# youngers2006/Dreamer

Hardware: AMD Instinct MI355X
Metric: imagined latent-steps/sec (B×H) at 64×64 CarRacing, 1/2/4/8 MI355X (higher is better)
Workload: dtype f32; 1 GPU; Dreamer.train_Agent() with AC_epochs=1 (replay sample + warm start S/2 + H-step imagination + actor-critic update), B=256/GPU S=64 H=15 64x64x3, precision=fp32 (north-star batch per GPU); global_batch=256, seq_len=64, horizon=15, parallelism=dp1, precision=fp32

## Files before the change

dreamer_amd/csrc/engine.hip:

```cpp
#include "engine_util.h"
#include "scan.h"
#include "dream.h"
#include "bptt.h"


static bool s3_first_layer(const dr_dims* d, int M, int N, const float* h, long long ldh, const float* z,
                           long long ldz) {
  return d->precision != DR_PREC_BF16 && M >= 1024 && ldh < INT_MAX && ldz < INT_MAX &&
         op_gemm_nt_split3_supported(M, N, d->hidden + latent(d), h, (int)ldh, z, (int)ldz, d->hidden, N);
}

struct EncWs {
  float *x0, *a[DR_MAX_DEPTH], *wr[DR_MAX_DEPTH], *sk;
  long long sk_n;
  void* wproj;
  void* s3proj;
  float* s3part;
  size_t s3part_n;
};

static void enc_carve(Carve& c, const dr_dims* d, int n, EncWs& w) {
  memset(&w, 0, sizeof(w));
  if (d->obs_dim > 0) {
    const int F = enc_feat_dim(d);
// ... 230 lines not shown
  WS_CHECK(c, ws_bytes);
  const int L = latent(d), Hd = d->hidden, eh = d->enc_hidden;
  const int F = enc_feat_dim(d);
  const bool any_gru = (z_init != nullptr) || T > 1;
  if (any_gru) {
    DR_REQUIRE(wm->w_ih && wm->w_hh && wm->b_ih && wm->b_hh, "GRU weights required");
    DR_TRY(op_transpose(3 * Hd, L + d->action, wm->w_ih, w.wt, s));
  }
  if (z_init == nullptr && h_init == nullptr && op_pscan_supported(d, B, T, d->action)) {
    const int rc = op_pscan(d, wm, B, T, d->action, feat, actions, act_sb, act_st, w.wt, wm->map0.w + F, F + Hd,
                            noise, 0, z_out, h_out, logits_out, w.ring, s);
    if (rc != DR_E_UNSUPPORTED) return rc;
  }
  return observe_steps(d, wm, B, T, feat, actions, act_sb, act_st, h_init, z_init, noise, z_out, h_out, logits_out, w,
                       nullptr, s);
}

static int observe_steps(const dr_dims* d, const dr_world_model* wm, int B, int T, const float* feat,
                         const float* actions, long long act_sb, long long act_st, const float* h_init,
                         const float* z_init, const dr_noise& noise, float* z_out, float* h_out, float* logits_out,
                         ObsWs& w, const ObsTrace* tr, hipStream_t s) {
  const int L = latent(d), Hd = d->hidden, eh = d->enc_hidden;
  const int F = enc_feat_dim(d);
  const long long ldL = (long long)T * L, ldH = (long long)T * Hd;
  const bool planes = B >= 128 && T > 1 && Hd % 8 == 0;
  if (planes) {
    DR_TRY(split_planes(eh, Hd, wm->map0.w + F, F + Hd, w.s3m0, s));
    DR_TRY(split_planes(3 * Hd, Hd, wm->w_hh, Hd, w.s3whh, s));
  }
  const float* h = h_init;
  const unsigned short* h16 = nullptr;
  const bool a16 = planes && d->precision == DR_PREC_BF16;
  int hb = 0;
  const bool split_gru = B >= 128;
  bool gh_pre = false;
  if (z_init) {
    if (z_init != z_out) DR_TRY(copy2d(z_out, L, z_init, L, L, B, s));
    DR_TRY(op_onehot_index(B, d->rows, d->cols, z_out, L, w.idx, onehot_vals(w.idx, B, d->rows), s));
    if (split_gru && planes && h_init) {
      GemmArgs gh = lin(B, 3 * Hd, Hd, h_init, Hd, wm->w_hh, Hd, wm->b_hh, w.gh, 3 * Hd);
      wplanes(gh, w.s3whh);
      DR_TRY(gemm_launch(G_NT, AM_PLAIN, &gh, 1, s));
      gh_pre = true;
    }
  }
  for (int t = 0; t < T; ++t) {
    const bool do_gru = (z_init != nullptr) || t > 0;
    if (do_gru) {
      const int ai = t - (z_init == nullptr ? 1 : 0);
      float* hn = w.hb[hb];
      unsigned short* hn16 = a16 ? w.hb16[hb] : nullptr;
      hb ^= 1;
      DR_TRY(gru_onehot(d, wm, B, w.idx, actions + ai * act_st, act_sb, h, Hd, hn, Hd, w.wt, nullptr,
                        nullptr, nullptr, nullptr, s, z_out, L, w.gh, gh_pre, hn16));
      h = hn;
      h16 = hn16;
    }
    GemmArgs g[2];
    g[0] = lin(B, eh, h ? Hd : 0, h, Hd, wm->map0.w + F, F + Hd, nullptr, w.pre1, eh);
    g[0].addend = feat + (long long)t * B * eh;
    g[0].ld_add = eh;
    const GemmArgs g_last = g[0];
    gh_pre = split_gru && h && t + 1 < T;
    if (gh_pre) {
      g[1] = lin(B, 3 * Hd, Hd, h, Hd, wm->w_hh, Hd, wm->b_hh, w.gh, 3 * Hd);
      if (planes) {
        wplanes(g[0], w.s3m0);
        wplanes(g[1], w.s3whh);
        g[0].A16 = g[1].A16 = h16;
      } else {
        g[0].bf16 = g[1].bf16 = 0;
      }
    }
    DR_TRY(gemm_launch(G_NT, AM_PLAIN, g, gh_pre ? 2 : 1, s));
    float* lg = (t == T - 1 && logits_out) ? logits_out : nullptr;
    long long ld_lg = L;
    const bool dual = tr && gh_pre && (planes || d->precision == DR_PREC_BF16);
    if (tr && tr->post_logits) {
      lg = tr->post_logits + (long long)t * L;
      ld_lg = ldL;
    }
    GemmArgs gp = lin_ln(B, L, eh, w.pre1, eh, wm->map1, wm->map3.w, wm->map3.b, dual ? nullptr : lg, ld_lg);
    with_sampler(gp, d, noise, t, z_out, L, w.idx, nullptr, 0);
    DR_TRY(run(G_NT, AM_LNSILU, gp, s));
    const float* zs = z_out;
    if (dual) {
      DR_TRY(gemm_launch(G_NT, AM_PLAIN, &g_last, 1, s));
      GemmArgs gq = lin_ln(B, L, eh, w.pre1, eh, wm->map1, wm->map3.w, wm->map3.b, lg, ld_lg);
      with_sampler(gq, d, noise, t, tr->z_last, L, tr->idx_last, nullptr, 0);
      DR_TRY(run(G_NT, AM_LNSILU, gq, s));
      zs = tr->z_last;
    }
    if (tr) {
      const float* hs = h;
      if (!hs) {
        DR_TRY(zero(w.hb[0], (long long)B * Hd, s));
        hs = w.hb[0];
      }
      const Copy2dJob cj[2] = {{tr->latents + (long long)t * L, ldL, zs, L, L, B},
                               {tr->hiddens + (long long)t * Hd, ldH, hs, Hd, Hd, B}};
      DR_TRY(op_copy2d_multi(cj, 2, s));
    }
  }
  if (!h_out) return DR_OK;
  if (h) DR_TRY(copy2d(h_out, Hd, h, Hd, Hd, B, s));
  else DR_TRY(zero(h_out, (long long)B * Hd, s));
  return DR_OK;
}

struct Tape {
  float *eps, *ls_raw;
  float *pre1a, *x1a, *pre2a, *x2a;
  float *r, *u, *n, *ghn;
  float *pre1p, *pre2p, *soft;
};
static void tape_carve(Carve& c, const dr_dims* d, int B, int H, Tape& t) {
  const long long BH = (long long)B * H;
  t.eps = c.f(BH * d->action);
  t.ls_raw = c.f(BH * d->action);
  t.pre1a = c.f(BH * d->actor_h1);
  t.x1a = c.f(BH * d->actor_h1);
  t.pre2a = c.f(BH * d->actor_h2);
  t.x2a = c.f(BH * d->actor_h2);
  t.r = c.f(BH * d->hidden);
  t.u = c.f(BH * d->hidden);
  t.n = c.f(BH * d->hidden);
  t.ghn = c.f(BH * d->hidden);
  t.pre1p = c.f(BH * d->prior_h1);
  t.pre2p = c.f(BH * d->prior_h2);
  t.soft = c.f(BH * latent(d));
}

extern "C" size_t dr_imagine_tape_bytes(const dr_dims* d, int B, int H) {
  Carve c(nullptr);
  Tape t;
  tape_carve(c, d, B, H, t);
  return c.off;
}

struct ImWs {
  float *gi, *gh, *plog, *p1r, *p1c, *p2r, *p2c, *rlog, *clog, *rval, *wt, *wst, *bst;
  unsigned short* hid16;
  float *tl0f, *hpart;
  void *s3r, *s3c;
  void *s3p0, *s3a0, *s3whh, *s3wt, *s3twhh, *s3tl0a;
  float* s3part;
  size_t s3part_n;
  int* idx[2];
  float *gH, *gZ, *gA, *glog, *gx2, *gp2, *gx1, *gp1, *ggi, *ggh, *gheads, *gx2a, *gpre2a, *gy2a, *xh2a, *gx1a,
      *gpre1a, *gy1a, *xh1a, *hcat, *zcat, *sk;
  unsigned short *ggi16, *ggh16, *gpre1a16;
  long long sk_n;
  float *tl6p, *tl3p, *tl0p, *twhh, *thead, *tl3a, *tl0a;
  void* tn;
  size_t tn_bytes;
  void* pd;
  void* pb;
};
static void imws_carve(Carve& c, const dr_dims* d, int B, int H, ImWs& w) {
  const long long Bl = B, BH = (long long)B * H, B1 = (long long)B * (H + 1);
  const int L = latent(d), Hd = d->hidden, A = d->action;
  w.gi = c.f(Bl * 3 * Hd);
  w.gh = c.f(Bl * 3 * Hd);
  w.plog = c.f(Bl * L);
  w.p1r = c.f(B1 * d->rew_h1);
  w.p1c = c.f(B1 * d->cont_h1);
  w.p2r = c.f(B1 * d->rew_h2);
  w.p2c = c.f(B1 * d->cont_h2);
  w.rlog = c.f(B1 * d->buckets);
  w.clog = c.f(B1);
  w.rval = c.f(B1);
  w.s3p0 = c.raw(op_nt_split3_ws_bytes(d->prior_h1, Hd));
  w.s3a0 = c.raw(op_nt_split3_ws_bytes(d->actor_h1, Hd));
  w.s3whh = c.raw(op_nt_split3_ws_bytes(3 * Hd, Hd));
  w.s3wt = c.raw(op_nt_split3_ws_bytes(L + A, 3 * Hd));
  w.s3twhh = c.raw(op_nt_split3_ws_bytes(Hd, 3 * Hd));
  w.s3tl0a = c.raw(op_nt_split3_ws_bytes(Hd + L, d->actor_h1));
  w.s3r = c.raw(op_nt_split3_ws_bytes(d->rew_h1, d->hidden + L));
  w.s3c = c.raw(op_nt_split3_ws_bytes(d->cont_h1, d->hidden + L));
  w.s3part_n = op_gemm_nt_split3_part_floats((int)B1, std::max(d->rew_h1, d->cont_h1));
  w.s3part = c.f((long long)w.s3part_n);
  w.wt = c.f((long long)(L + A) * 3 * Hd);
  w.hid16 = (unsigned short*)c.raw(sizeof(unsigned short) * Bl * (H + 1) * Hd);
  w.tl0f = c.f((long long)(Hd + L) * d->actor_h1);
  w.hpart = c.f(Bl * d->actor_h1);
  w.wst = c.f((long long)2 * A * d->actor_h2);
  w.bst = c.f((long long)2 * A);
  w.idx[0] = c.i(2 * Bl * d->rows);
  w.idx[1] = c.i(2 * Bl * d->rows);
  w.tl6p = c.f((long long)L * d->prior_h2);
  w.tl3p = c.f((long long)d->prior_h2 * d->prior_h1);
  w.tl0p = c.f((long long)d->prior_h1 * Hd);
  w.twhh = c.f((long long)3 * Hd * Hd);
  w.thead = c.f((long long)2 * A * d->actor_h2);
  w.tl3a = c.f((long long)d->actor_h2 * d->actor_h1);
  w.tl0a = c.f((long long)d->actor_h1 * (Hd + L));
  w.gH = c.f(B1 * Hd);
  w.gZ = c.f(B1 * L);
  w.gA = c.f(BH * A);
  w.glog = c.f(Bl * L);
  w.gx2 = c.f(Bl * d->prior_h2);
  w.gp2 = c.f(Bl * d->prior_h2);
  w.gx1 = c.f(Bl * d->prior_h1);
  w.gp1 = c.f(Bl * d->prior_h1);
  w.ggi = c.f(Bl * 3 * Hd);
  w.ggh = c.f(Bl * 3 * Hd);
  w.ggi16 = (unsigned short*)c.raw(sizeof(unsigned short) * Bl * 3 * Hd);
  w.ggh16 = (unsigned short*)c.raw(sizeof(unsigned short) * Bl * 3 * Hd);
  w.gheads = c.f(BH * 2 * A);
  w.gx2a = c.f(Bl * d->actor_h2);
  w.gpre2a = c.f(BH * d->actor_h2);
  w.gy2a = c.f(BH * d->actor_h2);
  w.xh2a = c.f(BH * d->actor_h2);
  w.gx1a = c.f(Bl * d->actor_h1);
  w.gpre1a = c.f(BH * d->actor_h1);
  w.gpre1a16 = (unsigned short*)c.raw(sizeof(unsigned short) * BH * d->actor_h1);
  w.gy1a = c.f(BH * d->actor_h1);
  w.xh1a = c.f(BH * d->actor_h1);
  w.hcat = c.f(BH * Hd);
  w.zcat = c.f(BH * L);
  w.sk_n = splitk_floats(d->actor_h1, Hd + L) + splitk_floats(d->actor_h2, d->actor_h1) +
           2 * splitk_floats(A, d->actor_h2);
  w.sk = c.f(w.sk_n);
  const int BHi = (int)BH;
  w.tn_bytes = op_gemm_tn_split3_ws_bytes(d->actor_h1, Hd + L, BHi) +
               op_gemm_tn_split3_ws_bytes(d->actor_h2, d->actor_h1, BHi) +
               2 * op_gemm_tn_split3_ws_bytes(A, d->actor_h2, BHi);
  w.tn = c.raw(w.tn_bytes);
  w.pd = c.raw(op_pdream_ws_bytes(d, B, H));
  w.pb = c.raw(op_pbptt_ws_bytes(d, B, H));
}

extern "C" size_t dr_imagine_workspace_bytes(const dr_dims* d, int B, int H) {
  Carve c(nullptr);
  ImWs w;
  imws_carve(c, d, B, H, w);
  return c.off;
}

static int imagine_heads(const dr_dims* d, const dr_world_model* wm, int B, int H, const float* latents,
                         const float* hiddens, float* rewards, float* continues, ImWs& w, hipStream_t s,
                         bool keep0 = false);

static int imagine_launch_form(const dr_dims* d, const dr_world_model* wm, const dr_actor* ac, int B, int H,
                               const dr_noise& noise, const dr_noise& nq, int deterministic, float* latents,
                               float* hiddens, float* actions, float* mus, float* sigmas, const Tape& tp, ImWs& w,
                               bool split_gru, bool zg, hipStream_t s) {
  const int L = latent(d), Hd = d->hidden, A = d->action, a1 = d->actor_h1, a2 = d->actor_h2;
  const long long ldH = (long long)(H + 1) * Hd, ldL = (long long)(H + 1) * L, ldA = (long long)H * A;
  const long long lda1 = (long long)H * a1, lda2 = (long long)H * a2;
  const bool planes = split_gru && H > 1 && Hd % 8 == 0;
  const bool a16 = planes && d->precision == DR_PREC_BF16;
  if (planes) {
    DR_TRY(split_planes(d->prior_h1, Hd, wm->prior.l0.w, Hd, w.s3p0, s));
    if (zg) DR_TRY(split_planes(a1, Hd, ac->l0.w, Hd + L, w.s3a0, s));
    DR_TRY(split_planes(3 * Hd, Hd, wm->w_hh, Hd, w.s3whh, s));
  }

  {
    DR_TRY(run(G_NT, AM_PLAIN, lin2(B, a1, hiddens, ldH, Hd, latents, ldL, L, ac->l0.w, ac->l0.b, tp.pre1a, lda1), s));
    GemmArgs g = lin_ln(B, a2, a1, tp.pre1a, lda1, ac->n1, ac->l3.w, ac->l3.b, tp.pre2a, lda2);
    g.a_out = tp.x1a; g.ld_aout = lda1;
    DR_TRY(run(G_NT, AM_LNSILU, g, s));
  }
  DR_TRY(stack_heads(ac, A, a2, w.wst, w.bst, s));
  {
    GemmArgs h = lin_ln(B, 2 * A, a2, tp.pre2a, lda2, ac->n4, w.wst, w.bst, nullptr, 0);
    h.a_out = tp.x2a; h.ld_aout = lda2;
    with_actor_head(h, A, noise, 0, deterministic, actions, ldA, mus, ldA, sigmas, ldA, tp.eps, tp.ls_raw, ldA);
    DR_TRY(run(G_NT, AM_LNSILU, h, s));
  }
  for (int t = 0; t < H; ++t) {
    const long long hb = (long long)Hd * B * t;
    float* h_t = hiddens + (long long)t * Hd;
    float* h_n = hiddens + (long long)(t + 1) * Hd;
    float* z_t = latents + (long long)t * L;
    float* z_n = latents + (long long)(t + 1) * L;
    unsigned short* h_n16 = a16 ? w.hid16 + (long long)(t + 1) * Hd : nullptr;
    DR_TRY(gru_onehot(d, wm, B, w.idx[t & 1], actions + (long long)t * A, ldA, h_t, ldH, h_n, ldH, w.wt,
                      tp.r + hb, tp.u + hb, tp.n + hb, tp.ghn + hb, s, z_t, ldL, w.gh, split_gru && t > 0, h_n16));
    float* p1 = tp.pre1p + (long long)t * B * d->prior_h1;
    float* p2 = tp.pre2p + (long long)t * B * d->prior_h2;
    {
      const bool more = t + 1 < H;
      GemmArgs p[3];
      int np = 0;
      p[np] = lin(B, d->prior_h1, Hd, h_n, ldH, wm->prior.l0.w, Hd, wm->prior.l0.b, p1, d->prior_h1);
      if (planes) wplanes(p[np], w.s3p0);
      ++np;
      if (more && zg) {
        p[np] = lin(B, a1, Hd, h_n, ldH, ac->l0.w, Hd + L, ac->l0.b, w.hpart, a1);
        if (planes) wplanes(p[np], w.s3a0);
        ++np;
      }
      if (more && split_gru) {
        p[np] = lin(B, 3 * Hd, Hd, h_n, ldH, wm->w_hh, Hd, wm->b_hh, w.gh, 3 * Hd);
        if (planes) wplanes(p[np], w.s3whh);
        ++np;
      }
      for (int i = 0; i < np; ++i) {
        if (!planes) p[i].bf16 = 0;
        p[i].A16 = h_n16;
      }
      DR_TRY(gemm_launch(G_NT, AM_PLAIN, p, np, s));
    }
    DR_TRY(run(G_NT, AM_LNSILU, lin_ln(B, d->prior_h2, d->prior_h1, p1, d->prior_h1, wm->prior.n1, wm->prior.l3.w,
                                       wm->prior.l3.b, p2, d->prior_h2), s));
    GemmArgs g = lin_ln(B, L, d->prior_h2, p2, d->prior_h2, wm->prior.n4, wm->prior.l6.w, wm->prior.l6.b, nullptr, 0);
    with_sampler(g, d, nq, t, z_n, ldL, w.idx[(t + 1) & 1], tp.soft + (long long)t * B * L, L);
    DR_TRY(run(G_NT, AM_LNSILU, g, s));
    if (t + 1 < H) {
      const long long o1 = (long long)(t + 1) * a1, o2 = (long long)(t + 1) * a2, o = (long long)(t + 1) * A;
      if (zg) {
        int* ix = w.idx[(t + 1) & 1];
        DR_TRY(op_zgather_add(B, a1, d->rows, d->cols, ix, onehot_vals(ix, B, d->rows), z_n, ldL,
                              w.tl0f + (long long)Hd * a1, a1, w.hpart, a1, tp.pre1a + o1, lda1, s));
      } else {
        DR_TRY(run(G_NT, AM_PLAIN, lin2(B, a1, h_n, ldH, Hd, z_n, ldL, L, ac->l0.w, ac->l0.b, tp.pre1a + o1, lda1), s));
      }
      GemmArgs g3 = lin_ln(B, a2, a1, tp.pre1a + o1, lda1, ac->n1, ac->l3.w, ac->l3.b, tp.pre2a + o2, lda2);
      g3.a_out = tp.x1a + o1;
      g3.ld_aout = lda1;
      DR_TRY(run(G_NT, AM_LNSILU, g3, s));
      GemmArgs hd = lin_ln(B, 2 * A, a2, tp.pre2a + o2, lda2, ac->n4, w.wst, w.bst, nullptr, 0);
      hd.a_out = tp.x2a + o2;
      hd.ld_aout = lda2;
      with_actor_head(hd, A, noise, t + 1, deterministic, actions + o, ldA, mus + o, ldA, sigmas + o, ldA,
                      tp.eps + (long long)(t + 1) * B * A, tp.ls_raw + o, ldA);
      DR_TRY(run(G_NT, AM_LNSILU, hd, s));
    }
  }
  return DR_OK;
}

extern "C" int dr_imagine_fwd(const dr_dims* d, const dr_world_model* wm, const dr_actor* ac, int B, int H,
                              const float* z0, const float* h0, dr_noise noise, int deterministic, float* latents,
                              float* hiddens, float* actions, float* rewards, float* continues, float* mus,
                              float* sigmas, void* tape, void* ws, size_t ws_bytes, hipStream_t s) {
  DR_REQUIRE(d && wm && ac && z0 && h0 && latents && hiddens && actions && rewards && continues && mus && sigmas &&
                 tape && B > 0 && H > 0,
             "null argument or empty batch");
  DR_TRY(dims_envelope(__func__, d, ENV_GRU | ENV_SAMPLER | ENV_ACTOR));
  GemmBf16Scope bf16_scope(d->precision == DR_PREC_BF16);
  Carve c(ws);
  ImWs w;
  imws_carve(c, d, B, H, w);
  WS_CHECK(c, ws_bytes);
  Carve ct(tape);
  Tape tp;
// ... 45 lines not shown
                                  w.p1c, d->cont_h1, w.s3part, w.s3part_n, s));
    } else {
      p[0] = lin2(M1, d->rew_h1, hiddens, Hd, Hd, latents, L, L, wm->reward.l0.w, wm->reward.l0.b, w.p1r, d->rew_h1);
      p[1] = lin2(M1, d->cont_h1, hiddens, Hd, Hd, latents, L, L, wm->cont.l0.w, wm->cont.l0.b, w.p1c, d->cont_h1);
      DR_TRY(gemm_launch(G_NT, AM_PLAIN, p, 2, s));
    }
    p[0] = lin_ln(M1, d->buckets, d->rew_h2, w.p2r, d->rew_h2, wm->reward.n4, wm->reward.l6.w, wm->reward.l6.b, w.rlog,
                  d->buckets);
    p[1] = lin_ln(M1, 1, d->cont_h2, w.p2c, d->cont_h2, wm->cont.n4, wm->cont.l6.w, wm->cont.l6.b, w.clog, 1);
    p[1].act = 2;
    Mlp2Args m2[2];
    {
      const float* x1[2] = {w.p1r, w.p1c};
      const dr_mlp3* hm[2] = {&wm->reward, &wm->cont};
      const int k1[2] = {d->rew_h1, d->cont_h1}, k2[2] = {d->rew_h2, d->cont_h2};
      for (int i = 0; i < 2; ++i) {
        memset(&m2[i], 0, sizeof(Mlp2Args));
        m2[i].M = M1; m2[i].K1 = k1[i]; m2[i].K2 = k2[i];
        m2[i].X = x1[i]; m2[i].ldx = k1[i];
        m2[i].ln1_g = hm[i]->n1.w; m2[i].ln1_b = hm[i]->n1.b;
        m2[i].W3 = hm[i]->l3.w; m2[i].b3 = hm[i]->l3.b;
        m2[i].ln4_g = hm[i]->n4.w; m2[i].ln4_b = hm[i]->n4.b;
        m2[i].e = p[i];
        m2[i].e.A = nullptr;
      }
    }
    if (mlp2_ok(m2[0]) && mlp2_ok(m2[1])) {
      DR_TRY(mlp2_launch(m2, 2, s));
    } else {
      GemmArgs q[2];
      q[0] = lin_ln(M1, d->rew_h2, d->rew_h1, w.p1r, d->rew_h1, wm->reward.n1, wm->reward.l3.w, wm->reward.l3.b, w.p2r,
                    d->rew_h2);
      q[1] = lin_ln(M1, d->cont_h2, d->cont_h1, w.p1c, d->cont_h1, wm->cont.n1, wm->cont.l3.w, wm->cont.l3.b, w.p2c,
                    d->cont_h2);
      DR_TRY(gemm_launch(G_NT, AM_LNSILU, q, 2, s));
      DR_TRY(gemm_launch(G_NT, AM_LNSILU, p, 2, s));
    }
    DR_TRY(op_bucket_value(M1, d->buckets, w.rlog, d->buckets, wm->buckets_rew, w.rval, 1, s));
    const int k0 = keep0 ? 0 : 1, Ho = H + 1 - k0;
    const Copy2dJob cj[2] = {{rewards, Ho, w.rval + k0, H + 1, Ho, B}, {continues, Ho, w.clog + k0, H + 1, Ho, B}};
    DR_TRY(op_copy2d_multi(cj, 2, s));
  }
  return DR_OK;
}

struct ImActWs {
  ImWs w;
  float *p1, *p2;
};
static void imact_carve(Carve& c, const dr_dims* d, int B, int H, ImActWs& a) {
  const long long Bl = B, B1 = (long long)B * (H + 1);
  const int L = latent(d), Hd = d->hidden, A = d->action;
  ImWs& w = a.w;
  memset(&w, 0, sizeof(w));
  w.gh = c.f(Bl * 3 * Hd);
  w.wt = c.f((long long)(L + A) * 3 * Hd);
  w.hid16 = (unsigned short*)c.raw(sizeof(unsigned short) * B1 * Hd);
  w.s3p0 = c.raw(op_nt_split3_ws_bytes(d->prior_h1, Hd));
  w.s3whh = c.raw(op_nt_split3_ws_bytes(3 * Hd, Hd));
  w.idx[0] = c.i(2 * Bl * d->rows);
  w.idx[1] = c.i(2 * Bl * d->rows);
  a.p1 = c.f(Bl * d->prior_h1);
  a.p2 = c.f(Bl * d->prior_h2);
  w.p1r = c.f(B1 * d->rew_h1);
  w.p1c = c.f(B1 * d->cont_h1);
  w.p2r = c.f(B1 * d->rew_h2);
  w.p2c = c.f(B1 * d->cont_h2);
  w.rlog = c.f(B1 * d->buckets);
  w.clog = c.f(B1);
  w.rval = c.f(B1);
  w.s3r = c.raw(op_nt_split3_ws_bytes(d->rew_h1, Hd + L));
  w.s3c = c.raw(op_nt_split3_ws_bytes(d->cont_h1, Hd + L));
  w.s3part_n = op_gemm_nt_split3_part_floats((int)B1, std::max(d->rew_h1, d->cont_h1));
  w.s3part = c.f((long long)w.s3part_n);
}

extern "C" size_t dr_imagine_actions_workspace_bytes(const dr_dims* d, int B, int H) {
  if (!d || B <= 0 || H <= 0) return 0;
  Carve c(nullptr);
  ImActWs a;
  imact_carve(c, d, B, H, a);
  return c.off;
}

extern "C" int dr_imagine_actions(const dr_dims* d, const dr_world_model* wm, int B, int H, const float* z0,
                                  const float* h0, const float* actions, long long act_sb, long long act_st,
                                  dr_noise noise, float* latents, float* hiddens, float* rewards, float* continues,
                                  void* ws, size_t ws_bytes, hipStream_t s) {
  DR_REQUIRE(d && wm && z0 && h0 && actions && latents && hiddens && rewards && continues && ws && B > 0 && H > 0,
             "null argument or empty batch");
  DR_REQUIRE(wm->w_ih && wm->w_hh && wm->b_ih && wm->b_hh, "GRU weights required");
  DR_TRY(dims_envelope(__func__, d, ENV_GRU | ENV_SAMPLER));
  GemmBf16Scope bf16_scope(d->precision == DR_PREC_BF16);
  Carve c(ws);
  ImActWs a;
  imact_carve(c, d, B, H, a);
  WS_CHECK(c, ws_bytes);
  ImWs& w = a.w;
  const int L = latent(d), Hd = d->hidden, A = d->action;
  const long long ldH = (long long)(H + 1) * Hd, ldL = (long long)(H + 1) * L;
  {
    const Copy2dJob cj[2] = {{latents, ldL, z0, L, L, B}, {hiddens, ldH, h0, Hd, Hd, B}};
    DR_TRY(op_copy2d_multi(cj, 2, s));
  }
  const bool split_gru = B >= 128;
  const bool planes = split_gru && H > 1 && Hd % 8 == 0;
  const bool a16 = planes && d->precision == DR_PREC_BF16;
  DR_TRY(op_transpose(3 * Hd, L + A, wm->w_ih, w.wt, s));
  DR_TRY(op_onehot_index(B, d->rows, d->cols, latents, ldL, w.idx[0], onehot_vals(w.idx[0], B, d->rows), s));
  if (planes) {
    DR_TRY(split_planes(d->prior_h1, Hd, wm->prior.l0.w, Hd, w.s3p0, s));
    DR_TRY(split_planes(3 * Hd, Hd, wm->w_hh, Hd, w.s3whh, s));
  }
  for (int t = 0; t < H; ++t) {
    float* h_t = hiddens + (long long)t * Hd;
    float* h_n = hiddens + (long long)(t + 1) * Hd;
    float* z_t = latents + (long long)t * L;
    float* z_n = latents + (long long)(t + 1) * L;
    unsigned short* h_n16 = a16 ? w.hid16 + (long long)(t + 1) * Hd : nullptr;
    DR_TRY(gru_onehot(d, wm, B, w.idx[t & 1], actions + (long long)t * act_st, act_sb, h_t, ldH, h_n, ldH, w.wt,
                      nullptr, nullptr, nullptr, nullptr, s, z_t, ldL, w.gh, split_gru && t > 0, h_n16));
    {
      GemmArgs p[2];
      int np = 0;
      p[np] = lin(B, d->prior_h1, Hd, h_n, ldH, wm->prior.l0.w, Hd, wm->prior.l0.b, a.p1, d->prior_h1);
      if (planes) wplanes(p[np], w.s3p0);
      ++np;
      if (t + 1 < H && split_gru) {
        p[np] = lin(B, 3 * Hd, Hd, h_n, ldH, wm->w_hh, Hd, wm->b_hh, w.gh, 3 * Hd);
        if (planes) wplanes(p[np], w.s3whh);
        ++np;
      }
      for (int i = 0; i < np; ++i) {
        if (!planes) p[i].bf16 = 0;
        p[i].A16 = h_n16;
      }
      DR_TRY(gemm_launch(G_NT, AM_PLAIN, p, np, s));
    }
    DR_TRY(run(G_NT, AM_LNSILU, lin_ln(B, d->prior_h2, d->prior_h1, a.p1, d->prior_h1, wm->prior.n1, wm->prior.l3.w,
                                       wm->prior.l3.b, a.p2, d->prior_h2), s));
    GemmArgs g = lin_ln(B, L, d->prior_h2, a.p2, d->prior_h2, wm->prior.n4, wm->prior.l6.w, wm->prior.l6.b, nullptr, 0);
    with_sampler(g, d, noise, t, z_n, ldL, w.idx[(t + 1) & 1], nullptr, 0);
    DR_TRY(run(G_NT, AM_LNSILU, g, s));
  }
  return imagine_heads(d, wm, B, H, latents, hiddens, rewards, continues, w, s);
}

static int imagine_bwd_impl(const dr_dims* d, const dr_world_model* wm, const dr_actor* ac, int B, int H,
                            const float* latents, const float* hiddens, const float* actions,
                            const float* g_mus, const float* g_sigmas,
                            const float* g_actions, const float* g_latents, const float* g_hiddens,
                            const void* tape, const dr_actor* gr, void* ws, size_t ws_bytes, hipStream_t s,
                            bool do_prep, bool do_main);

extern "C" int dr_imagine_bwd(const dr_dims* d, const dr_world_model* wm, const dr_actor* ac, int B, int H,
                              const float* latents, const float* hiddens, const float* actions,
                              const float* g_mus, const float* g_sigmas,
                              const float* g_actions, const float* g_latents, const float* g_hiddens,
                              const void* tape, const dr_actor* gr, void* ws, size_t ws_bytes, hipStream_t s) {
  return imagine_bwd_impl(d, wm, ac, B, H, latents, hiddens, actions, g_mus, g_sigmas, g_actions, g_latents,
                          g_hiddens, tape, gr, ws, ws_bytes, s, true, true);
}

extern "C" int dr_imagine_bwd_prep(const dr_dims* d, const dr_world_model* wm, const dr_actor* ac, int B, int H,
                                   const float* g_actions, const float* g_latents, const float* g_hiddens, void* ws,
                                   size_t ws_bytes, hipStream_t s) {
  DR_REQUIRE(d && wm && ac && B > 0 && H > 0, "null argument or empty batch");
  return imagine_bwd_impl(d, wm, ac, B, H, nullptr, nullptr, nullptr, nullptr, nullptr, g_actions, g_latents,
                          g_hiddens, nullptr, nullptr, ws, ws_bytes, s, true, false);
}

extern "C" int dr_imagine_bwd_main(const dr_dims* d, const dr_world_model* wm, const dr_actor* ac, int B, int H,
                                   const float* latents, const float* hiddens, const float* actions,
                                   const float* g_mus, const float* g_sigmas, int upstream_state, const void* tape,
                                   const dr_actor* gr, void* ws, size_t ws_bytes, hipStream_t s) {
  const float* flag = upstream_state ? reinterpret_cast<const float*>(ws) : nullptr;
  return imagine_bwd_impl(d, wm, ac, B, H, latents, hiddens, actions, g_mus, g_sigmas, nullptr, flag, nullptr, tape,
                          gr, ws, ws_bytes, s, false, true);
}

static int imagine_bwd_impl(const dr_dims* d, const dr_world_model* wm, const dr_actor* ac, int B, int H,
                            const float* latents, const float* hiddens, const float* actions,
                            const float* g_mus, const float* g_sigmas,
                            const float* g_actions, const float* g_latents, const float* g_hiddens,
                            const void* tape, const dr_actor* gr, void* ws, size_t ws_bytes, hipStream_t s,
                            bool do_prep, bool do_main) {
  DR_REQUIRE(d && wm && ac && B > 0 && H > 0, "null argument or empty batch");
  DR_TRY(dims_envelope("dr_imagine_bwd", d, ENV_GRU | ENV_SAMPLER | ENV_ACTOR));
  GemmBf16Scope bf16_scope(d->precision == DR_PREC_BF16);
  DR_REQUIRE(!do_main || (latents && hiddens && actions && tape && gr), "null argument");
  Carve c(ws);
  ImWs w;
  imws_carve(c, d, B, H, w);
  WS_CHECK(c, ws_bytes);
  Carve ct((void*)tape);
  Tape tp;
  if (do_main) tape_carve(ct, d, B, H, tp);
  const int L = latent(d), Hd = d->hidden, A = d->action, a1 = d->actor_h1, a2 = d->actor_h2;
  const long long ldH = (long long)(H + 1) * Hd, ldL = (long long)(H + 1) * L, ldA = (long long)H * A;
  const long long lda1 = (long long)H * a1, lda2 = (long long)H * a2;
  const int BH = B * H;
  const bool upstream_state = g_latents || g_hiddens;
  if (do_prep) {
  if (!g_hiddens && !g_latents && !g_actions) {
    DR_TRY(zero(w.gH, (long long)((w.gA + (long long)BH * A) - w.gH), s));
  } else {
    if (g_hiddens) DR_TRY(copy2d(w.gH, Hd, g_hiddens, Hd, Hd, (long long)B * (H + 1), s));
    else DR_TRY(zero(w.gH, (long long)B * (H + 1) * Hd, s));
    if (g_latents) DR_TRY(copy2d(w.gZ, L, g_latents, L, L, (long long)B * (H + 1), s));
    else DR_TRY(zero(w.gZ, (long long)B * (H + 1) * L, s));
    if (g_actions) DR_TRY(copy2d(w.gA, A, g_actions, A, A, (long long)BH, s));
    else DR_TRY(zero(w.gA, (long long)BH * A, s));
  }
  {
    const int h1 = d->prior_h1, h2 = d->prior_h2;
    TransposeJob tj[9] = {
        {L, h2, L, wm->prior.l6.w, w.tl6p},
        {h2, h1, h2, wm->prior.l3.w, w.tl3p},
        {h1, Hd, h1, wm->prior.l0.w, w.tl0p},
        {3 * Hd, L + A, 3 * Hd, wm->w_ih, w.wt},
        {3 * Hd, Hd, 3 * Hd, wm->w_hh, w.twhh},
        {A, a2, 2 * A, ac->mu.w, w.thead},
        {A, a2, 2 * A, ac->ls.w, w.thead + A},
        {a2, a1, a2, ac->l3.w, w.tl3a},
        {a1, Hd + L, a1, ac->l0.w, w.tl0a},
    };
    DR_TRY(op_transpose_multi(tj, 9, s));
    if (B >= 128 && (3 * Hd) % 8 == 0) {
      DR_TRY(split_planes(L + A, 3 * Hd, w.wt, 3 * Hd, w.s3wt, s));
      DR_TRY(split_planes(Hd, 3 * Hd, w.twhh, 3 * Hd, w.s3twhh, s));
      if (d->actor_h1 % 8 == 0) DR_TRY(split_planes(Hd + L, d->actor_h1, w.tl0a, d->actor_h1, w.s3tl0a, s));
    }
  }
  }
  const bool planes = B >= 128 && (3 * Hd) % 8 == 0;
  if (!do_main) return DR_OK;

  bool looped = false;
  if (op_pbptt_supported(d, B, H, A)) {
    const PBpttIO io = {w.tl6p, w.tl3p, w.tl0p, w.wt, w.twhh, w.thead, w.tl3a, w.tl0a,
                        tp.soft, tp.pre2p, tp.pre1p, tp.r, tp.u, tp.n, tp.ghn, tp.pre2a, tp.pre1a, tp.ls_raw, tp.eps,
                        hiddens, actions, g_mus, g_sigmas, w.gH, w.gZ, w.gA,
                        w.gheads, w.gpre2a, w.gy2a, w.xh2a, w.gpre1a, w.gy1a, w.xh1a};
    const int rc = op_pbptt(d, wm, ac, B, H, io, w.pb, s);
    if (rc != DR_E_UNSUPPORTED && rc != DR_OK) return rc;
    looped = rc == DR_OK;
  }
  for (int t = H - 1; t >= 0 && !looped; --t) {
    const long long hb = (long long)Hd * B * t;
    float* gH_t = w.gH + (long long)t * Hd;
    float* gH_n = w.gH + (long long)(t + 1) * Hd;
    float* gZ_t = w.gZ + (long long)t * L;
    float* gZ_n = w.gZ + (long long)(t + 1) * L;
    const bool state_grad = upstream_state || t < H - 1;
    if (state_grad) {
      const int h1 = d->prior_h1, h2 = d->prior_h2;
      GemmArgs g = bwd_nt(B, h2, L, gZ_n, ldL, w.tl6p, w.gx2, h2, 0);
      g.pre = tp.soft + (long long)t * B * L;
      g.ld_pre = L;
      g.C = d->cols;
      const GemmPlan pl = gemm_plan(G_NT, AM_STEBWD, &g, 1);
      if (gemm_bwd_fusable(pl)) {
        DR_TRY(gemm_run(pl, &g, 1, s));
      } else {
        DR_TRY(op_softmax_ste_bwd(B, d->rows, d->cols, gZ_n, ldL, tp.soft + (long long)t * B * L, L, w.glog, s));
        DR_TRY(run(G_NT, AM_PLAIN, bwd_nt(B, h2, L, w.glog, L, w.tl6p, w.gx2, h2, 0), s));
      }
      DR_TRY(lnbwd_nt(B, h1, h2, w.gx2, h2, tp.pre2p + (long long)t * B * h2, h2, wm->prior.n4, w.tl3p, w.gx1, h1, 0,
                      w.gp2, h2, nullptr, nullptr, nullptr, 0, INT_MAX, s));
      GruBwdEpi ge;
      memset(&ge, 0, sizeof(ge));
      ge.h = hiddens + (long long)t * Hd; ge.ldh = ldH;
      ge.r = tp.r + hb; ge.u = tp.u + hb; ge.n = tp.n + hb; ge.ghn = tp.ghn + hb;
      ge.gi = w.ggi; ge.gh = w.ggh; ge.ho = gH_t; ge.ldo = ldH; ge.Hd = Hd;
      const bool a16 = planes && d->precision == DR_PREC_BF16;
      if (a16) {
        ge.gi16 = w.ggi16;
        ge.gh16 = w.ggh16;
      }
      DR_TRY(lnbwd_nt(B, Hd, h1, w.gx1, h1, tp.pre1p + (long long)t * B * h1, h1, wm->prior.n1, w.tl0p, gH_n, ldH, 1,
                      w.gp1, h1, nullptr, nullptr, nullptr, 0, INT_MAX, s, &ge));
      if (t > 0) {
        GemmArgs p[2];
        p[0] = bwd_nt(B, L + A, 3 * Hd, w.ggi, 3 * Hd, w.wt, gZ_t, ldL, 1);
        p[0].Y2 = w.gA + (long long)t * A; p[0].ldy2 = ldA; p[0].nsplitY = L;
        p[1] = bwd_nt(B, Hd, 3 * Hd, w.ggh, 3 * Hd, w.twhh, gH_t, ldH, 1);
        if (planes) {
          wplanes(p[0], w.s3wt);
          wplanes(p[1], w.s3twhh);
        }
        if (a16) {
          p[0].A16 = w.ggi16;
          p[1].A16 = w.ggh16;
        }
        DR_TRY(gemm_launch(G_NT, AM_PLAIN, p, 2, s));
      } else {
        DR_TRY(run(G_NT, AM_PLAIN, bwd_nt(B, A, 3 * Hd, w.ggi, 3 * Hd, w.wt + (long long)L * 3 * Hd, w.gA, ldA, 1), s));
      }
    }
    const long long ot = (long long)t * A;
    float* gh_t = w.gheads + (long long)t * 2 * A;
    const long long o2 = (long long)t * a2, o1 = (long long)t * a1;
    DR_TRY(op_actor_head_bwd_x(B, A, a2, w.gA + ot, ldA, g_mus ? g_mus + ot : nullptr,
                               g_sigmas ? g_sigmas + ot : nullptr, ldA, actions + ot, ldA, tp.ls_raw + ot, ldA,
                               tp.eps + (long long)t * B * A, gh_t, (long long)H * 2 * A, w.thead, w.gx2a, a2, s));
    DR_TRY(lnbwd_nt(B, a1, a2, w.gx2a, a2, tp.pre2a + o2, lda2, ac->n4, w.tl3a, w.gx1a, a1, 0, w.gpre2a + o2, lda2,
                    w.gy2a + o2, w.xh2a + o2, nullptr, 0, INT_MAX, s));
    if (t > 0 && planes && a1 % 8 == 0) {
      const bool a16 = d->precision == DR_PREC_BF16 && lda1 % 8 == 0;
      DR_TRY(op_ln_silu_bwd(B, a1, w.gx1a, a1, tp.pre1a + o1, lda1, ac->n1.w, ac->n1.b, w.gpre1a + o1, lda1,
                            w.gy1a + o1, w.xh1a + o1, s, a16 ? w.gpre1a16 + o1 : nullptr));
      GemmArgs g = bwd_nt(B, Hd + L, a1, w.gpre1a + o1, lda1, w.tl0a, gH_t, ldH, 1);
      if (a16) g.A16 = w.gpre1a16 + o1;
      g.Y2 = gZ_t; g.ldy2 = ldL; g.nsplitY = Hd;
      wplanes(g, w.s3tl0a);
      DR_TRY(run(G_NT, AM_PLAIN, g, s));
    } else if (t > 0) {
      DR_TRY(lnbwd_nt(B, Hd + L, a1, w.gx1a, a1, tp.pre1a + o1, lda1, ac->n1, w.tl0a, gH_t, ldH, 1, w.gpre1a + o1,
                      lda1, w.gy1a + o1, w.xh1a + o1, gZ_t, ldL, Hd, s));
    } else {
      DR_TRY(op_ln_silu_bwd(B, a1, w.gx1a, a1, tp.pre1a + o1, lda1, ac->n1.w, ac->n1.b, w.gpre1a + o1, lda1,
                            w.gy1a + o1, w.xh1a + o1, s));
    }
  }
  {
    const Copy2dJob cj[2] = {{w.hcat, (long long)H * Hd, hiddens, ldH, (long long)H * Hd, B},
                             {w.zcat, (long long)H * L, latents, ldL, (long long)H * L, B}};
    DR_TRY(op_copy2d_multi(cj, 2, s));
  }
  {
    GemmArgs p[4];
    p[0] = bwd_w(a1, Hd + L, BH, w.gpre1a, a1, w.hcat, Hd, gr->l0.w);
    p[0].W2 = w.zcat; p[0].ldb2 = L; p[0].nsplitB = Hd;
    p[1] = bwd_w(a2, a1, BH, w.gpre2a, a2, tp.x1a, a1, gr->l3.w);
    p[2] = bwd_w(A, a2, BH, w.gheads, 2 * A, tp.x2a, a2, gr->mu.w);
    p[3] = bwd_w(A, a2, BH, w.gheads + A, 2 * A, tp.x2a, a2, gr->ls.w);
    float* sk = w.sk;
    long long skn = w.sk_n;
    for (int i = 0; i < 4; ++i) give_splitk(p[i], sk, skn);
    DR_TRY(tn_launch(p, 4, w.tn, w.tn_bytes, s, d->precision == DR_PREC_BF16 ? 1 : 3));
  }
  {
    ColsumJob cj[8] = {
        {a1, w.gpre1a, a1, nullptr, 0, gr->l0.b}, {a1, w.gy1a, a1, w.xh1a, a1, gr->n1.w},
        {a1, w.gy1a, a1, nullptr, 0, gr->n1.b},   {a2, w.gpre2a, a2, nullptr, 0, gr->l3.b},
        {a2, w.gy2a, a2, w.xh2a, a2, gr->n4.w},   {a2, w.gy2a, a2, nullptr, 0, gr->n4.b},
        {A, w.gheads, 2 * A, nullptr, 0, gr->mu.b}, {A, w.gheads + A, 2 * A, nullptr, 0, gr->ls.b},
    };
    DR_TRY(op_colsum_multi(BH, cj, 8, s));
  }
  return DR_OK;
}

struct CTape {
  float *pre1, *x1, *pre2, *x2, *logits;
};
static void ctape_carve(Carve& c, const dr_dims* d, int M, CTape& t) {
  t.pre1 = c.f((long long)M * d->critic_h1);
  t.x1 = c.f((long long)M * d->critic_h1);
  t.pre2 = c.f((long long)M * d->critic_h2);
  t.x2 = c.f((long long)M * d->critic_h2);
  t.logits = c.f((long long)M * d->buckets);
}

extern "C" size_t dr_critic_tape_bytes(const dr_dims* d, int M) {
  Carve c(nullptr);
  CTape t;
  ctape_carve(c, d, M, t);
  return c.off;
}

static size_t critic_ws_bytes(const dr_dims* d, int M) {
  Carve c(nullptr);
  CTape t;
  ctape_carve(c, d, M, t);
  c.f(splitk_floats(M, d->critic_h1));
  c.raw(op_nt_split3_ws_bytes(d->critic_h1, d->hidden + latent(d)));
  c.f((long long)op_gemm_nt_split3_part_floats(M, d->critic_h1));
  return c.off + 256;
}


extern "C" int dr_critic_fwd(const dr_dims* d, const dr_critic* cr, int M, const float* h, long long ldh,
                             const float* z, long long ldz, float* logits, float* values, void* tape, void* ws,
                             size_t ws_bytes, hipStream_t s) {
  DR_REQUIRE(d && cr && h && z && M > 0, "null argument or empty batch");
  GemmBf16Scope bf16_scope(d->precision == DR_PREC_BF16);
  CTape t;
  float* sk = nullptr;
  long long skn = 0;
  void* s3w = nullptr;
  float* s3part = nullptr;
  size_t s3part_n = 0;
  if (tape) {
    Carve c(tape);
    ctape_carve(c, d, M, t);
  }
  if (ws) {
    Carve c(ws);
    CTape tw;
    ctape_carve(c, d, M, tw);
    if (!tape) {
      t = tw;
      WS_CHECK(c, ws_bytes);
    }
    const long long want = splitk_floats(M, d->critic_h1);
    if (c.off + (size_t)want * sizeof(float) + 256 <= ws_bytes) {
      skn = want;
      sk = c.f(skn);
      const size_t pb = op_nt_split3_ws_bytes(d->critic_h1, d->hidden + latent(d));
      if (c.off + pb + 256 <= ws_bytes) s3w = c.raw(pb);
      const size_t pn = op_gemm_nt_split3_part_floats(M, d->critic_h1);
      if (s3w && c.off + pn * sizeof(float) + 256 <= ws_bytes) {
        s3part = c.f((long long)pn);
        s3part_n = pn;
      }
    }
  }
  DR_REQUIRE(tape || ws, "dr_critic_fwd needs a tape or a workspace");
  const int L = latent(d), Hd = d->hidden, c1 = d->critic_h1, c2 = d->critic_h2, nb = d->buckets;
  if (s3w && s3_first_layer(d, M, c1, h, ldh, z, ldz)) {
    DR_TRY(op_nt_repack_split3(c1, Hd + L, cr->net.l0.w, Hd + L, s3w, s));
    DR_TRY(op_gemm_nt_split3_sk(M, c1, Hd + L, h, (int)ldh, z, (int)ldz, Hd, s3w, cr->net.l0.b, 0, t.pre1, c1,
                                s3part, s3part_n, s));
  } else {
    GemmArgs g1 = lin2(M, c1, h, ldh, Hd, z, ldz, L, cr->net.l0.w, cr->net.l0.b, t.pre1, c1);
    give_splitk(g1, sk, skn);
    DR_TRY(run(G_NT, AM_PLAIN, g1, s));
  }
  GemmArgs g2 = lin_ln(M, c2, c1, t.pre1, c1, cr->net.n1, cr->net.l3.w, cr->net.l3.b, t.pre2, c2);
  g2.a_out = t.x1; g2.ld_aout = c1;
  DR_TRY(run(G_NT, AM_LNSILU, g2, s));
  float* lg = logits ? logits : t.logits;
  GemmArgs g3 = lin_ln(M, nb, c2, t.pre2, c2, cr->net.n4, cr->net.l6.w, cr->net.l6.b, lg, nb);
  g3.a_out = t.x2; g3.ld_aout = c2;
  DR_TRY(run(G_NT, AM_LNSILU, g3, s));
  if (tape && logits && logits != t.logits) DR_TRY(copy2d(t.logits, nb, logits, nb, nb, M, s));
  if (values) DR_TRY(op_bucket_value(M, nb, lg, nb, cr->buckets, values, 1, s));
  return DR_OK;
}

struct CBws {
  float *row_loss, *glog, *gx2, *gp2, *gy2, *xh2, *gx1, *gp1, *gy1, *xh1;
  float *tl6, *tl3;
  float* sk;
  long long sk_n;
  void* tn;
  size_t tn_bytes;
};
static void cbws_carve(Carve& c, const dr_dims* d, int B, int H, CBws& w) {
  const long long M = (long long)B * (H + 1);
  w.tn_bytes = op_gemm_tn_split3_ws_bytes(d->buckets, d->critic_h2, (int)M) +
               op_gemm_tn_split3_ws_bytes(d->critic_h2, d->critic_h1, (int)M) +
               op_gemm_tn_split3_ws_bytes(d->critic_h1, d->hidden + latent(d), (int)M);
  w.tn = c.raw(w.tn_bytes);
  w.row_loss = c.f((long long)B * H);
  w.sk_n = splitk_floats(d->buckets, d->critic_h2) + splitk_floats(d->critic_h2, d->critic_h1) +
           splitk_floats(d->critic_h1, d->hidden + latent(d));
  w.sk = c.f(w.sk_n);
  w.tl6 = c.f((long long)d->buckets * d->critic_h2);
  w.tl3 = c.f((long long)d->critic_h2 * d->critic_h1);
  w.glog = c.f(M * d->buckets);
  w.gx2 = c.f(M * d->critic_h2);
  w.gp2 = c.f(M * d->critic_h2);
  w.gy2 = c.f(M * d->critic_h2);
  w.xh2 = c.f(M * d->critic_h2);
  w.gx1 = c.f(M * d->critic_h1);
  w.gp1 = c.f(M * d->critic_h1);
  w.gy1 = c.f(M * d->critic_h1);
// ... 249 lines not shown
```

dreamer_amd/csrc/gemm.h:

```cpp
#pragma once
#include "common.h"

enum { AM_PLAIN = 0, AM_LNSILU = 1, AM_CONV = 2, AM_CONV_SRC = 3, AM_LNBWD = 4, AM_STEBWD = 5 };

struct GruBwdEpi {
  const float* h; long long ldh;
  const float *r, *u, *n, *ghn;
  float *gi, *gh;
  float* ho; long long ldo;
  int Hd, pad_;
  unsigned short *gi16, *gh16;
};

struct alignas(16) GemmArgs {
  int M, N, K;
  const float* A; long long lda;
  const float* A2; long long lda2; int ksplitA;
  const float* ln_g; const float* ln_b;
  float* a_out; long long ld_aout;
  const float* pre; long long ld_pre;
  float* splitk_ws; long long splitk_floats;
  float* sv_gy; float* sv_xh; long long ld_sv;
  int cin, ih, iw, oh, ow;
  dr_frames src;
  int nb;
  const float* W; long long ldb;
  const float* W2; long long ldb2; int ksplitB; int nsplitB;
  const float* bias; const float* addend; long long ld_add;
  float* Y; long long ldy;
  float* Y2; long long ldy2; int nsplitY;
  int accumulate, act, out_conv;
  float alpha;
  int epi;
  dr_noise noise; int step;
  int R, C; float unimix;
  float* z_out; long long ldz; int* idx_out; float* soft_out; long long ld_soft;
  float* zval_out;
  int na, det;
  float* act_out; long long ld_act; float* mu_out; long long ld_mu; float* sig_out; long long ld_sig;
  float* eps_save; float* ls_save; long long ld_ls;
  int bf16;
  GruBwdEpi gb;
  const unsigned short* wsplit; int wsplit_np, pad2_;
  const unsigned short* A16;
};

enum { EPI_NONE = 0, EPI_SAMPLE = 1, EPI_ACTOR = 2 };

enum GemmLayout { G_NT = 0, G_NN = 1, G_TN = 2 };

GemmArgs gemm_args();
struct GemmBf16Scope {
  explicit GemmBf16Scope(bool on);
  ~GemmBf16Scope();
  int prev;
};
int gemm_launch(GemmLayout lay, int amode, const GemmArgs* probs, int count, hipStream_t s);

enum GemmFamily {
  GF_LEGACY = 0,
  GF_SKINNY,
  GF_TILE,
  GF_TILE_B16,
  GF_WK,
  GF_WKS3,
  GF_LN_SAMPLE,
  GF_S3_TALL,
  GF_LN_ROWS,
  GF_SPLITK_FINISH
};
struct GemmStep {
  int family, bm, bn, kc, nw, amode, a_km, b_kn, vec, epi, bf16, a16;
  int mask;
  int gx, gy, gz, block, lds;
  int splits, npack, no_ws;
};
struct GemmPlan {
  int rc; char err[192];
  int ln_pre, nsteps;
  GemmStep step[10];
};
GemmPlan gemm_plan(GemmLayout lay, int amode, const GemmArgs* probs, int count);
int gemm_run(const GemmPlan& pl, const GemmArgs* probs, int count, hipStream_t s);
int gemm_bwd_fusable(const GemmPlan& pl);

struct alignas(16) Mlp2Args {
  int M, K1, K2, pad_;
  const float* X; long long ldx;
  const float* ln1_g; const float* ln1_b;
  const float* W3; const float* b3;
  const float* ln4_g; const float* ln4_b;
  float* a1_out; long long ld_a1;
  float* pre2; long long ld_pre2;
  float* a2_out; long long ld_a2;
  GemmArgs e;
};
bool mlp2_ok(const Mlp2Args& a);
int mlp2_launch(const Mlp2Args* probs, int count, hipStream_t s);
```

dreamer_amd/csrc/gemm.hip:

```cpp
#include <limits.h>
#include <stdarg.h>
#include <stdio.h>
#include <stdlib.h>
#include <stdint.h>
#include <string.h>

#include "gemm.h"
#include "conv.h"

#include <algorithm>

#define BK 32
#define LDS_K (BK + 2)

struct GemmBatch {
  GemmArgs p[4];
};

template <int BM, int BN>
__device__ __forceinline__ int dr_pack_tile(const GemmBatch& gb, int npack, int& z) {
  z = blockIdx.z;
  if (npack <= 0) return -2;
  int tot = 0;
  for (int i = 0; i < npack; ++i) tot += ((gb.p[i].M + BM - 1) / BM) * ((gb.p[i].N + BN - 1) / BN);
// ... 1537 lines not shown
    lt = dr_xcd_tile(blockIdx.x, tot);
    if (lt < 0) return;
    z = 0;
    for (int i = 0; i + 1 < npack; ++i) {
      const int ti = ((gb.p[i].M + BM - 1) / BM) * ((gb.p[i].N + BN - 1) / BN);
      if (lt < ti) break;
      lt -= ti;
      z = i + 1;
    }
  }
  dr_stage_args(gb.p[z], s_args, threadIdx.x);
  const GemmArgs& g = s_args;
  const int M = dr_uni(g.M), N = dr_uni(g.N), K = dr_uni(g.K);
  const int tiles_m = (M + BM - 1) / BM, tiles_n = (N + BN - 1) / BN;
  if (npack == 0) lt = dr_xcd_tile(blockIdx.x, tiles_m * tiles_n);
  if (lt < 0) return;
  const int tn = lt / tiles_m, tm = lt - tn * tiles_m;
  const int m0 = tm * BM, n0 = tn * BN;
  const int tid = threadIdx.x, wave = tid >> 6, lane = tid & 63;
  const int r = lane & 15, q = lane >> 4;
  const float* A = dr_uni(g.A);
  const float* A2 = dr_uni(g.A2);
  const float* W = dr_uni(g.W);
  const int lda = dr_uni((int)g.lda), lda2 = dr_uni((int)g.lda2), ldb = dr_uni((int)g.ldb);
  const int ksA = dr_uni(g.ksplitA);

  constexpr int NEPI = (NT4 + NTH - 1) / NTH;
  float ebias[NEPI];
  {
    const float* bias = dr_uni(g.bias);
#pragma unroll
    for (int i = 0; i < NEPI; ++i) {
      const int x = tid + NTH * i, l = x & 63, tj = x >> 8;
      const int n = n0 + (tj % FN) * 16 + (l & 15);
      const bool ok = bias && splits == 1 && x < NT4 && n < N;
      const float v = dr_ld1(ok ? bias : W, ok ? (unsigned)n : 0u);
      ebias[i] = ok ? v : 0.f;
    }
  }

  const int nkb = (K + 31) >> 5;
  const int per = (nkb + splits - 1) / splits;
  const int kb0 = min(nkb, (int)blockIdx.y * per), kb1 = min(nkb, kb0 + per);
  const int nbg = kb1 - kb0;
  const int b0 = kb0 + (nbg * wave) / NW, b1 = kb0 + (nbg * (wave + 1)) / NW;
  const int blast = max(min(b1, nkb) - 1, 0);

  unsigned oa[FM], oa2[FM], ob[FN];
#pragma unroll
  for (int i = 0; i < FM; ++i) {
    const int m = min(m0 + 16 * i + r, M - 1);
    oa[i] = (unsigned)(m * lda);
    oa2[i] = (unsigned)(m * lda2);
  }
#pragma unroll
  for (int j = 0; j < FN; ++j) ob[j] = (unsigned)(min(n0 + 16 * j + r, N - 1) * ldb);

  f32x4 ra[D][FM][2], rb[D][FN][2];
  constexpr int KL = KMAP == 0 ? 8 : 4, KH = KMAP == 0 ? 4 : 16;
  auto load = [&](int b, int sl) {
#pragma unroll
    for (int h = 0; h < 2; ++h) {
      const int k = 32 * b + KL * q + KH * h;
      const int kk = k < K ? k : 0;
      const bool s1 = kk < ksA;
#pragma unroll
      for (int i = 0; i < FM; ++i) {
        const float* base = s1 ? A : A2;
        const unsigned e = s1 ? oa[i] + (unsigned)kk : oa2[i] + (unsigned)(kk - ksA);
        ra[sl][i][h] = *(const DR_GLOBAL f32x4*)((const DR_GLOBAL char*)base + (e << 2));
      }
#pragma unroll
      for (int j = 0; j < FN; ++j) {
        const unsigned e = ob[j] + (unsigned)kk;
        rb[sl][j][h] = *(const DR_GLOBAL f32x4*)((const DR_GLOBAL char*)W + (e << 2));
      }
    }
  };
  f32x4 acc[1][FM][FN];
#pragma unroll
  for (int i = 0; i < FM; ++i)
#pragma unroll
    for (int j = 0; j < FN; ++j) acc[0][i][j] = (f32x4){0.f, 0.f, 0.f, 0.f};
#pragma unroll
  for (int u = 0; u < D; ++u) load(min(b0 + u, blast), u);
  const int nbw = b1 - b0;
  const bool ktail = (K & 31) != 0;
  for (int bb = 0; bb < nbw; bb += D) {
#pragma unroll
    for (int u = 0; u < D; ++u) {
      if (bb + u >= nbw) break;
      const int b = b0 + bb + u;
      if (ktail && b == nkb - 1) {
#pragma unroll
        for (int h = 0; h < 2; ++h) {
          if (32 * b + KL * q + KH * h < K) continue;
#pragma unroll
          for (int i = 0; i < FM; ++i) ra[u][i][h] = (f32x4){0.f, 0.f, 0.f, 0.f};
#pragma unroll
          for (int j = 0; j < FN; ++j) rb[u][j][h] = (f32x4){0.f, 0.f, 0.f, 0.f};
        }
      }
#pragma unroll
      for (int h = 0; h < 2; ++h)
#pragma unroll
        for (int c = 0; c < 4; ++c)
#pragma unroll
          for (int i = 0; i < FM; ++i)
#pragma unroll
            for (int j = 0; j < FN; ++j)
              acc[0][i][j] =
                  __builtin_amdgcn_mfma_f32_16x16x4f32(ra[u][i][h][c], rb[u][j][h][c], acc[0][i][j], 0, 0, 0);
      load(min(b + D, blast), u);
    }
  }
#pragma unroll
  for (int i = 0; i < FM; ++i)
#pragma unroll
    for (int j = 0; j < FN; ++j) {
      const f32x4 v = acc[0][i][j];
#pragma unroll
      for (int e = 0; e < 4; ++e) red[wave][(i * FN + j) * 4 + e][lane] = v[e];
    }
  __syncthreads();
  float* part = g.splitk_ws;
#pragma unroll
  for (int ii = 0; ii < NEPI; ++ii) {
    const int x = tid + NTH * ii;
    if (x >= NT4) break;
    const int l = x & 63, e = (x >> 6) & 3, tj = x >> 8;
    float v = 0.f;
#pragma unroll
    for (int w = 0; w < NW; ++w) v += red[w][tj * 4 + e][l];
    const int t = tj / FN, j = tj - t * FN;
    const int m = m0 + t * 16 + 4 * (l >> 4) + e, n = n0 + j * 16 + (l & 15);
    if (m >= M || n >= N) continue;
    if (splits == 1) epilogue_store_b(g, m, n, v, ebias[ii]);
    else dr_g(part)[((long long)blockIdx.y * M + m) * N + n] = v;
  }
}

typedef unsigned wk_u32x4 __attribute__((ext_vector_type(4)));
typedef __bf16 wk_bf16x8 __attribute__((ext_vector_type(8)));
__device__ __forceinline__ f32x4 wk_mfma(wk_u32x4 a, wk_u32x4 b, f32x4 c) {
  return __builtin_amdgcn_mfma_f32_16x16x32_bf16(__builtin_bit_cast(wk_bf16x8, a), __builtin_bit_cast(wk_bf16x8, b),
                                                  c, 0, 0, 0);
}
__device__ __forceinline__ unsigned wk_pack_rne(float x0, float x1) {
  typedef __bf16 b2 __attribute__((ext_vector_type(2)));
  const b2 v = {(__bf16)x0, (__bf16)x1};
  return __builtin_bit_cast(unsigned, v);
}

template <int NTP, int D, int NW = 4, int FM = 2, bool A16 = false>
__global__ __launch_bounds__(64 * NW) void k_gemm_wks3(GemmBatch gb, int npack) {
  static_assert(!A16 || NTP == 1, "bf16 A copies feed the one-term form only");
  constexpr int FN = 2, BM = 16 * FM, NTH = 64 * NW, NT4 = FM * FN * 256;
  __shared__ GemmArgs s_args;
  __shared__ __attribute__((aligned(16))) float red[NW][FM * FN * 4][64];
  int z = 0;
  const int plt = dr_pack_tile<BM, 32>(gb, npack, z);
  if (plt == -1) return;
  dr_stage_args(gb.p[z], s_args, threadIdx.x);
  const GemmArgs& g = s_args;
  const int M = dr_uni(g.M), N = dr_uni(g.N), K = dr_uni(g.K);
  const int tiles_m = (M + BM - 1) / BM, tiles_n = (N + 31) / 32;
  const int lt = plt >= 0 ? plt : dr_xcd_tile(blockIdx.x, tiles_m * tiles_n);
  if (lt < 0) return;
  const int tn = lt / tiles_m, tm = lt - tn * tiles_m;
  const int m0 = tm * BM, n0 = tn * 32;
  const int tid = threadIdx.x, wave = tid >> 6, lane = tid & 63, r = lane & 15, q = lane >> 4;
  const float* A = dr_uni(g.A);
  const unsigned short* A16p = dr_uni(g.A16);
  const int lda = dr_uni((int)g.lda);
  const unsigned short* wr = dr_uni(g.wsplit);
  const int Np = dr_uni(g.wsplit_np);
  constexpr int NEPI = (NT4 + NTH - 1) / NTH;
  float ebias[NEPI];
  {
    const float* bias = dr_uni(g.bias);
#pragma unroll
    for (int i = 0; i < NEPI; ++i) {
      const int x = tid + NTH * i, l = x & 63, e = (x >> 6) & 3, tj = x >> 8;
      const int n = n0 + (tj % FN) * 16 + 4 * (l >> 4) + e;
      const bool ok = bias && x < NT4 && n < N;
      ebias[i] = ok ? dr_ld1(bias, (unsigned)n) : 0.f;
    }
  }
  const int nkc = (K + 31) >> 5;
  const int c0 = (nkc * wave) / NW, c1 = (nkc * (wave + 1)) / NW;
  const int clast = max(c1 - 1, 0);
  unsigned oa[FM];
#pragma unroll
  for (int i = 0; i < FM; ++i) oa[i] = (unsigned)(min(m0 + 16 * i + r, M - 1) * lda);
  unsigned ob[FN];
#pragma unroll
  for (int j = 0; j < FN; ++j) ob[j] = (unsigned)(n0 + 16 * j + r) * 32u + 8u * q;
  f32x4 ra[A16 ? 1 : D][FM][2];
  wk_u32x4 ra16[A16 ? D : 1][FM];
  wk_u32x4 rb[D][NTP][FN];
  auto load = [&](int c, int sl) {
    const int k = 32 * c + 8 * q;
    const unsigned kk = k < K ? (unsigned)k : 0u;
#pragma unroll
    for (int i = 0; i < FM; ++i) {
      if constexpr (A16) {
        ra16[sl][i] = *(const DR_GLOBAL wk_u32x4*)((const DR_GLOBAL char*)A16p + ((oa[i] + kk) << 1));
      } else {
        ra[sl][i][0] = *(const DR_GLOBAL f32x4*)((const DR_GLOBAL char*)A + ((oa[i] + kk) << 2));
        ra[sl][i][1] = *(const DR_GLOBAL f32x4*)((const DR_GLOBAL char*)A + ((oa[i] + kk + 4) << 2));
      }
    }
#pragma unroll
    for (int p = 0; p < NTP; ++p)
#pragma unroll
      for (int j = 0; j < FN; ++j) {
        const unsigned e = (unsigned)((c * 3 + p) * Np) * 32u + ob[j];
        rb[sl][p][j] = *(const DR_GLOBAL wk_u32x4*)((const DR_GLOBAL char*)wr + (e << 1));
      }
  };
  constexpr int NA = 1;
  f32x4 acc[NA][FM][FN];
#pragma unroll
  for (int a3 = 0; a3 < NA; ++a3)
#pragma unroll
    for (int i = 0; i < FM; ++i)
#pragma unroll
      for (int j = 0; j < FN; ++j) acc[a3][i][j] = (f32x4){0.f, 0.f, 0.f, 0.f};
#pragma unroll
  for (int u = 0; u < D; ++u) load(min(c0 + u, clast), u);
  const int ncw = c1 - c0;
  for (int cc = 0; cc < ncw; cc += D) {
#pragma unroll
    for (int u = 0; u < D; ++u) {
      if (cc + u >= ncw) break;
      const int c = c0 + cc + u;
      const bool kin = 32 * c + 8 * q < K;
      wk_u32x4 a[NTP][FM];
#pragma unroll
      for (int i = 0; i < FM; ++i) {
        if constexpr (A16) {
          a[0][i] = kin ? ra16[u][i] : (wk_u32x4){0u, 0u, 0u, 0u};
          continue;
        }
        f32x4 x0 = ra[A16 ? 0 : u][i][0], x1 = ra[A16 ? 0 : u][i][1];
        if (!kin) x0 = x1 = (f32x4){0.f, 0.f, 0.f, 0.f};
        if constexpr (NTP == 3) {
          unsigned h[4], m[4], l[4];
          split3_pair(x0[0], x0[1], h[0], m[0], l[0]);
          split3_pair(x0[2], x0[3], h[1], m[1], l[1]);
          split3_pair(x1[0], x1[1], h[2], m[2], l[2]);
          split3_pair(x1[2], x1[3], h[3], m[3], l[3]);
          a[0][i] = (wk_u32x4){h[0], h[1], h[2], h[3]};
          a[1 % NTP][i] = (wk_u32x4){m[0], m[1], m[2], m[3]};
          a[2 % NTP][i] = (wk_u32x4){l[0], l[1], l[2], l[3]};
        } else {
          a[0][i] = (wk_u32x4){wk_pack_rne(x0[0], x0[1]), wk_pack_rne(x0[2], x0[3]), wk_pack_rne(x1[0], x1[1]),
                               wk_pack_rne(x1[2], x1[3])};
        }
      }
#define DR_WK3(PA, PB, X)                        \
  _Pragma("unroll") for (int i = 0; i < FM; ++i) _Pragma("unroll") for (int j = 0; j < FN; ++j) acc[X][i][j] = \
      wk_mfma(rb[u][PB][j], a[PA][i], acc[X][i][j]);
      if constexpr (NTP == 3) {
        DR_WK3(2 % NTP, 0, 0)
        DR_WK3(1 % NTP, 1 % NTP, 0)
        DR_WK3(0, 2 % NTP, 0)
        DR_WK3(1 % NTP, 0, 0)
        DR_WK3(0, 1 % NTP, 0)
      }
      DR_WK3(0, 0, 0)
#undef DR_WK3
      load(min(c + D, clast), u);
    }
  }
  {
#pragma unroll
    for (int i = 0; i < FM; ++i)
#pragma unroll
      for (int j = 0; j < FN; ++j) {
        const f32x4 v = acc[0][i][j];
#pragma unroll
        for (int e = 0; e < 4; ++e) red[wave][(i * FN + j) * 4 + e][lane] = v[e];
      }
  }
  __syncthreads();
#pragma unroll
  for (int ii = 0; ii < NEPI; ++ii) {
    const int x = tid + NTH * ii;
    if (x >= NT4) break;
    const int l = x & 63, e = (x >> 6) & 3, tj = x >> 8;
    float v = 0.f;
#pragma unroll
    for (int w = 0; w < NW; ++w) v += red[w][tj * 4 + e][l];
    const int t = tj / FN, j = tj - t * FN;
    const int m = m0 + t * 16 + (l & 15), n = n0 + j * 16 + 4 * (l >> 4) + e;
    if (m >= M || n >= N) continue;
    epilogue_store_b(g, m, n, v, ebias[ii]);
  }
}

__global__ __launch_bounds__(256) void k_splitk_finish(GemmBatch gb, int splits) {
  __shared__ GemmArgs s_args;
  dr_stage_args(gb.p[blockIdx.z], s_args, threadIdx.x);
  const GemmArgs& g = s_args;
  const long long MN = (long long)g.M * g.N;
  const long long i = (long long)blockIdx.x * 256 + threadIdx.x;
  if (i >= MN) return;
  float v = 0.f;
  for (int sp = 0; sp < splits; ++sp) v += dr_g(g.splitk_ws)[sp * MN + i];
  const int m = (int)(i / g.N), n = (int)(i - (long long)m * g.N);
  epilogue_store(g, m, n, v);
}

#define MLP2_KMAX 208
#define MLP2_NC 128
struct Mlp2Batch {
  Mlp2Args p[3];
};

__device__ __forceinline__ float4 mlp2_ln_silu(float4 x, bool ok, int K, const float* gam, const float* bet, int k) {
  const float mean = wave_sum(ok ? (x.x + x.y) + (x.z + x.w) : 0.f) / (float)K;
  float sq = 0.f;
  if (ok) {
    const float dx = x.x - mean, dy = x.y - mean, dz = x.z - mean, dw = x.w - mean;
    sq = (dx * dx + dy * dy) + (dz * dz + dw * dw);
  }
  const float rstd = 1.0f / sqrtf(wave_sum(sq) / (float)K + 1e-5f);
  if (!ok) return make_float4(0.f, 0.f, 0.f, 0.f);
  const float4 gv = dr_ld4(gam, (unsigned)k), bv = dr_ld4(bet, (unsigned)k);
  return make_float4(dr_silu_fast((x.x - mean) * rstd * gv.x + bv.x), dr_silu_fast((x.y - mean) * rstd * gv.y + bv.y),
                     dr_silu_fast((x.z - mean) * rstd * gv.z + bv.z), dr_silu_fast((x.w - mean) * rstd * gv.w + bv.w));
}

#define MLP2_KS (MLP2_KMAX / 16)
__device__ __forceinline__ void mlp2_wload(float4 (&wv)[MLP2_KS], const float* W, int ldw, int n, bool nok, int K,
                                           int q) {
  const int ks = (K + 15) >> 4;
#pragma unroll
  for (int s = 0; s < MLP2_KS; ++s) {
    const int k = 16 * s + 4 * q;
    const bool ok = s < ks && nok && k < K;
    wv[s] = dr_ld4(W, ok ? (unsigned)(n * ldw + k) : 0u);
    if (!ok) wv[s] = make_float4(0.f, 0.f, 0.f, 0.f);
  }
}
template <int LP>
__device__ __forceinline__ f32x4 mlp2_tile(const float (*ys)[LP], const float4 (&wv)[MLP2_KS], int K, int r, int q) {
  const int ks = (K + 15) >> 4;
  f32x4 c[4];
#pragma unroll
  for (int j = 0; j < 4; ++j) c[j] = (f32x4){0.f, 0.f, 0.f, 0.f};
#pragma unroll
  for (int s = 0; s < MLP2_KS; ++s) {
    if (s < ks) {
      const float4 a = *reinterpret_cast<const float4*>(&ys[r][16 * s + 4 * q]);
      c[s & 3] = __builtin_amdgcn_mfma_f32_16x16x4f32(a.x, wv[s].x, c[s & 3], 0, 0, 0);
      c[s & 3] = __builtin_amdgcn_mfma_f32_16x16x4f32(a.y, wv[s].y, c[s & 3], 0, 0, 0);
      c[s & 3] = __builtin_amdgcn_mfma_f32_16x16x4f32(a.z, wv[s].z, c[s & 3], 0, 0, 0);
// ... 224 lines not shown
  for (int i = 0; i < LNV; ++i) sm += (xv[i].x + xv[i].y) + (xv[i].z + xv[i].w);
  const float mean = wave_sum(sm) / (float)K;
  float sq = 0.f;
#pragma unroll
  for (int i = 0; i < LNV; ++i) {
    if (lane + 64 * i < K4) {
      const float dx = xv[i].x - mean, dy = xv[i].y - mean, dz = xv[i].z - mean, dw = xv[i].w - mean;
      sq += (dx * dx + dy * dy) + (dz * dz + dw * dw);
    }
  }
  const float rstd = 1.0f / sqrtf(wave_sum(sq) / (float)K + 1e-5f);
#pragma unroll
  for (int i = 0; i < LNV; ++i) {
    const int k4 = lane + 64 * i;
    if (k4 < K4) {
      float4 y;
      y.x = dr_silu_fast((xv[i].x - mean) * rstd * gv[i].x + bv[i].x);
      y.y = dr_silu_fast((xv[i].y - mean) * rstd * gv[i].y + bv[i].y);
      y.z = dr_silu_fast((xv[i].z - mean) * rstd * gv[i].z + bv[i].z);
      y.w = dr_silu_fast((xv[i].w - mean) * rstd * gv[i].w + bv[i].w);
      *reinterpret_cast<float4*>(Y + (long long)m * ldy + 4 * k4) = y;
    }
  }
}

static bool aligned16(const void* p) { return ((uintptr_t)p & 15) == 0; }
struct PlanProbs {
  const GemmArgs* p[4];
  int mask = 0, n = 0;
  void add(const GemmArgs* g, int i) { p[n++] = g; mask |= 1 << i; }
  const GemmArgs& operator[](int i) const { return *p[i]; }
};
static void plan_fail(GemmPlan& pl, const char* fmt, ...) {
  va_list ap;
  va_start(ap, fmt);
  vsnprintf(pl.err, sizeof(pl.err), fmt, ap);
  va_end(ap);
  pl.rc = DR_E_INVALID;
}
static GemmStep& plan_step(GemmPlan& pl, int family, int mask, int gx, int gy, int gz, int block) {
  GemmStep& st = pl.step[pl.nsteps++] = GemmStep{};
  st.family = family; st.mask = mask; st.gx = gx; st.gy = gy; st.gz = gz; st.block = block;
  return st;
}
static bool rows_aligned(const GemmArgs& g, int kq, bool a, bool w) {
  if (a && (g.K % kq != 0 || g.lda % 4 != 0 || !aligned16(g.A))) return false;
  if (a && g.ksplitA < g.K && (g.ksplitA % kq != 0 || g.lda2 % 4 != 0 || !aligned16(g.A2))) return false;
  return !w || (g.ldb % 4 == 0 && aligned16(g.W));
}
struct TileCount { int maxt, tot; bool ws; int maxM, minK; };
static TileCount tile_count(const PlanProbs& q, int bm, int bn) {
  TileCount c = {0, 0, true, 0, 1 << 30};
  for (int i = 0; i < q.n; ++i) {
    const int t = dr_cdiv(q[i].M, bm) * dr_cdiv(q[i].N, bn);
    c.maxt = std::max(c.maxt, t);
    c.tot += t;
    c.ws = c.ws && q[i].splitk_ws != nullptr;
    c.maxM = std::max(c.maxM, q[i].M);
    c.minK = std::min(c.minK, q[i].K);
  }
  return c;
}
static int splitk_count(const PlanProbs& q, int tot, int kc) {
  int nch = 1 << 30;
  for (int i = 0; i < q.n; ++i) nch = std::min(nch, dr_cdiv(q[i].K, kc));
  int splits = std::max(1, std::min(DR_TILE_SPLITS, dr_cdiv(512, tot)));
  splits = std::min(splits, std::max(1, nch / 2));
  for (int i = 0; i < q.n; ++i)
    while (splits > 1 && (long long)splits * q[i].M * q[i].N > q[i].splitk_floats) --splits;
  return splits;
}

static bool skinny_offsets_ok(const GemmArgs& g, bool b_kn) {
  const long long lim = 1LL << 30;
  return (long long)g.M * g.lda < lim && (long long)g.M * g.lda2 < lim && (long long)(b_kn ? g.K : g.N) * g.ldb < lim &&
         !(g.W2 && (long long)(g.K + g.N) * g.ldb2 >= lim) && !(g.a_out && (long long)g.M * g.ld_aout >= lim);
}

static int skinny_tile_rows(const PlanProbs& q, int amode, int maxM, bool sample) {
  if (maxM <= 64) return 16;
  if (amode != AM_PLAIN && amode != AM_LNSILU && amode != AM_LNBWD && amode != AM_STEBWD) return 64;
  return tile_count(q, 16, sample ? 32 : 16).tot <= 640 ? 16 : 64;
}

static bool plan_skinny(GemmPlan& pl, const PlanProbs& q, int amode, bool b_kn) {
  int maxM = 0, epi = EPI_NONE;
  bool vec = true;
  for (int i = 0; i < q.n; ++i) {
    const GemmArgs& g = q[i];
    if (g.out_conv) return false;
    if ((g.epi == EPI_SAMPLE) != (q[0].epi == EPI_SAMPLE)) return false;
    if (g.epi != EPI_NONE) epi = g.epi;
    maxM = g.M > maxM ? g.M : maxM;
    if (!skinny_offsets_ok(g, b_kn)) return false;
    vec = vec && rows_aligned(g, 4, true, !b_kn);
  }
  if (maxM > (epi == EPI_NONE ? (1 << 20) : 4096)) return false;
  const int mt = skinny_tile_rows(q, amode, maxM, epi == EPI_SAMPLE);
  bool wide = mt == 16 && tile_count(q, 16, 16).tot > 256;
  bool wide48 = false;
  if (amode == AM_LNBWD && epi == EPI_NONE && wide && vec) {
    const int t32 = tile_count(q, 16, 32).tot;
    wide48 = t32 > 256 && t32 < 512 && tile_count(q, 16, 48).tot <= 256;
    for (int i = 0; i < q.n; ++i) wide48 = wide48 && sk_staged(amode, 16, 48, q[i].K, vec, b_kn);
  }
  const bool bwd = amode == AM_LNBWD || amode == AM_STEBWD;
  if (bwd && wide && !wide48 && epi != EPI_SAMPLE)
    for (int i = 0; i < q.n; ++i) wide = wide && sk_staged(amode, 16, 32, q[i].K, vec, b_kn);
  const int nt = epi == EPI_SAMPLE ? 32 : (epi == EPI_ACTOR || mt == 64) ? 16 : wide48 ? 48 : wide ? 32 : 16;
  int lds = 0;
  for (int i = 0; i < q.n; ++i) {
    if (bwd && !sk_staged(amode, mt, nt, q[i].K, vec, b_kn)) return false;
    lds = std::max(lds, sk_lds_floats(amode, mt, nt, q[i].K, vec, b_kn));
  }
  const TileCount tc = tile_count(q, mt, nt);
  if (tc.maxt == 0) return true;
  const int npack = q.n > 1 ? q.n : 0;
  GemmStep& st =
      plan_step(pl, GF_SKINNY, q.mask, dr_xcd_grid(npack ? tc.tot : tc.maxt), 1, npack ? 1 : q.n, 64 * DR_SKW);
  st.bm = mt; st.bn = nt; st.amode = amode; st.b_kn = b_kn; st.vec = vec; st.epi = epi; st.npack = npack;
  st.lds = lds * (int)sizeof(float);
  return true;
}

static void plan_tile(GemmPlan& pl, const PlanProbs& q, int family, int bm, int bn, int kc, int nw, bool a_km,
                      bool b_kn, bool no_ws) {
  const TileCount tc = tile_count(q, bm, bn);
  if (tc.maxt == 0) return;
  const bool b16 = family == GF_TILE_B16;
  long long maxMN = 0;
  bool vec = true;
  for (int i = 0; i < q.n; ++i) {
    maxMN = std::max(maxMN, (long long)q[i].M * q[i].N);
    vec = vec && rows_aligned(q[i], 4, !a_km, !b_kn);
  }
  const int splits = (!no_ws && tc.ws && (!b16 || tc.tot < 256)) ? splitk_count(q, tc.tot, kc) : 1;
  const int npack = (!b16 && q.n > 1) ? q.n : 0;
  GemmStep& st = plan_step(pl, family, q.mask, dr_xcd_grid(npack ? tc.tot : tc.maxt), splits, npack ? 1 : q.n, 64 * nw);
  st.bm = bm; st.bn = bn; st.kc = kc; st.nw = nw; st.a_km = a_km; st.b_kn = b_kn; st.vec = b16 || vec; st.bf16 = b16;
  st.splits = splits; st.npack = npack; st.no_ws = no_ws;
  if (splits > 1) plan_step(pl, GF_SPLITK_FINISH, q.mask, (int)((maxMN + 255) / 256), 1, q.n, 256).splits = splits;
}

static bool chain_ok(const PlanProbs& q, bool b16) {
  for (int i = 0; i < q.n; ++i) {
    const GemmArgs& g = q[i];
    if (!rows_aligned(g, 8, true, true) || g.W2 || g.epi != EPI_NONE || g.out_conv) return false;
    if (b16 ? !g.bf16 : (g.K < 8 || g.M < 1 || g.N < 1)) return false;
  }
  return true;
}
static bool b16_ok(const PlanProbs& q) { return chain_ok(q, true); }

static bool wks3_ok(const PlanProbs& q) {
  for (int i = 0; i < q.n; ++i) {
    const GemmArgs& g = q[i];
    if (!g.wsplit || g.wsplit_np < ((g.N + 31) & ~31) || g.K < 8 || !rows_aligned(g, 8, true, false) ||
        ((uintptr_t)g.wsplit & 15) || g.ksplitA < g.K || g.W2 || g.epi != EPI_NONE || g.out_conv || g.M < 1 || g.N < 1 ||
        (long long)g.M * g.lda >= (1LL << 30) || (long long)((g.K + 31) / 32) * 3 * g.wsplit_np * 32 >= (1LL << 30))
      return false;
  }
  return true;
}
#define DR_WKS3_D 1
#define DR_WKS3_NW 4
#define DR_WKS3_FM 2
#define DR_WKS3_FM_B16 1
static void plan_wave(GemmPlan& pl, const PlanProbs& q, int family, bool bf16, bool no_ws) {
  const int fm = family == GF_WK ? 2 : bf16 ? DR_WKS3_FM_B16 : DR_WKS3_FM, nw = family == GF_WK ? 4 : DR_WKS3_NW;
  const TileCount tc = tile_count(q, 16 * fm, 32);
  if (tc.maxt == 0) return;
  const int npack = q.n > 1 ? q.n : 0;
  bool a16 = family == GF_WKS3 && bf16;
  for (int i = 0; i < q.n && a16; ++i) a16 = q[i].A16 && ((uintptr_t)q[i].A16 & 15) == 0 && q[i].lda % 8 == 0;
  GemmStep& st = plan_step(pl, family, q.mask, dr_xcd_grid(npack ? tc.tot : tc.maxt), 1, 1, 64 * nw);
  st.bm = 16 * fm; st.bn = 32; st.nw = nw; st.vec = 1; st.bf16 = family == GF_WKS3 && bf16; st.a16 = a16;
  st.splits = 1; st.npack = npack; st.no_ws = no_ws;
}

static bool tile_offsets_ok(const PlanProbs& q) {
  const long long lim = 1LL << 30;
  for (int i = 0; i < q.n; ++i) {
    const GemmArgs& g = q[i];
    const long long arows = std::max((long long)g.M, (long long)g.K), brows = std::max((long long)g.N, (long long)g.K);
    if (arows * g.lda >= lim || arows * g.lda2 >= lim || brows * g.ldb >= lim) return false;
    if (g.epi != EPI_NONE || g.out_conv) return false;
  }
  return true;
}

int op_gemm_nt_split3_ex(int M, int N, int K, const float* A, int lda, const float* A2, int lda2, int ksA,
                         const void* wr, const float* bias, int act, float* Y, int ldy, int accumulate, float* Y2,
                         int ldy2, int nsplitY, float* part, size_t part_floats, hipStream_t s, int splits_fixed);
static bool s3_tall_ok(const GemmArgs& g) {
  const bool seg = g.ksplitA < g.K;
  return g.wsplit && !g.bf16 && g.M >= 1024 && g.epi == EPI_NONE && !g.out_conv && !g.W2 && !g.addend &&
         g.alpha == 1.0f && (g.act == 0 || g.act == 1) &&
         (!seg || (g.A2 && aligned16(g.A2) && g.ksplitA % 4 == 0 && g.lda2 % 4 == 0 &&
                   (long long)g.M * g.lda2 < (1LL << 31))) &&
         g.wsplit_np == (g.N + 127) / 128 * 128 &&
         g.N % 4 == 0 && g.K % 4 == 0 && g.lda % 4 == 0 && g.ldy % 4 == 0 && aligned16(g.A) && aligned16(g.Y) &&
         (!g.bias || aligned16(g.bias)) && (g.nsplitY >= g.N || (g.Y2 && aligned16(g.Y2) && g.ldy2 % 4 == 0 &&
                                                                  g.nsplitY % 4 == 0)) &&
         (long long)g.M * g.lda < (1LL << 31) && g.lda < INT_MAX && g.ldy < INT_MAX && g.ldy2 < INT_MAX;
}

static void plan_route(GemmPlan& pl, int amode, bool a_km, bool b_kn, PlanProbs q) {
  const bool nt = !a_km && !b_kn;
  if (amode == AM_PLAIN && nt) {
    PlanProbs rest;
    for (int i = 0; i < q.n; ++i) {
      if (s3_tall_ok(q[i])) plan_step(pl, GF_S3_TALL, 1 << i, 0, 0, 0, 0);
      else rest.add(q.p[i], i);
    }
    if (rest.n == 0) return;
    q = rest;
  }
  if (amode == AM_PLAIN && tile_offsets_ok(q)) {
    const TileCount t64 = tile_count(q, 64, 64);
    const int maxM = t64.maxM, minK = t64.minK;
    const bool step_rows = nt && maxM >= 128 && maxM <= 512;
    if (step_rows && minK < 512 && wks3_ok(q)) return plan_wave(pl, q, GF_WKS3, b16_ok(q), false);
    if (step_rows) {
      const int tiles32 = tile_count(q, 32, 32).tot;
      if ((minK >= 1024 && (tiles32 >= 112 || b16_ok(q))) || (minK >= 512 && tiles32 >= 256)) {
        const bool no_ws = tiles32 >= 256;
        if (wks3_ok(q)) plan_wave(pl, q, GF_WKS3, b16_ok(q), no_ws);
        else if (b16_ok(q)) plan_tile(pl, q, GF_TILE_B16, 32, 32, 64, 4, false, false, no_ws);
        else if (chain_ok(q, false)) plan_wave(pl, q, GF_WK, false, no_ws);
        else plan_tile(pl, q, GF_TILE, 32, 32, 64, 4, false, false, no_ws);
        return;
      }
    }
    const bool tall = nt && maxM >= 1024 && t64.tot >= 256;
    if (a_km || (maxM >= 256 && minK >= 512 && (t64.ws || t64.tot >= 128)) || tall) {
      if (nt && minK >= 1024 && b16_ok(q)) plan_tile(pl, q, GF_TILE_B16, 64, 64, 64, 8, false, false, false);
      else if (nt && minK >= 1024) plan_tile(pl, q, GF_TILE, 64, 64, 64, 8, false, false, false);
      else plan_tile(pl, q, GF_TILE, 64, 64, 32, 4, a_km, b_kn, false);
      return;
    }
  }
  if (amode == AM_LNBWD || amode == AM_STEBWD) {
    if (nt && plan_skinny(pl, q, amode, false)) return;
    plan_fail(pl, amode == AM_LNBWD ? "gemm: LayerNorm-backward prologue needs the staged NT skinny path"
                                    : "gemm: softmax-STE-backward prologue needs the staged NT skinny path");
    return;
  }
  if (!a_km && (amode == AM_PLAIN || amode == AM_LNSILU) && plan_skinny(pl, q, amode, b_kn)) return;
  long long work = 0;
  for (int i = 0; i < q.n; ++i) work += (long long)q[i].M * q[i].N;
  const int bt = work >= 256LL * 1024 ? 64 : 32;
  const TileCount tc = tile_count(q, bt, bt);
  if (tc.maxt == 0) return;
  GemmStep& st = plan_step(pl, GF_LEGACY, q.mask, tc.maxt, 1, q.n, 256);
  st.bm = st.bn = bt; st.amode = amode; st.a_km = a_km; st.b_kn = b_kn;
}

static bool ln_sample_ok(const GemmArgs& g) {
  return g.epi == EPI_SAMPLE && g.C == 32 && g.R * g.C == g.N && g.N % LS_NT == 0 && g.K > 0 && g.K % 4 == 0 &&
         g.K <= LS_KMAX && g.M > 0 && g.M <= 65536 && g.ln_g && g.ln_b && g.ksplitA >= g.K && !g.addend &&
         g.alpha == 1.0f && g.act == 0 && !g.accumulate && !g.W2 && aligned16(g.A) && aligned16(g.W) &&
         aligned16(g.ln_g) && aligned16(g.ln_b) && g.lda % 4 == 0 && g.ldb % 4 == 0 &&
         (!g.a_out || (aligned16(g.a_out) && g.ld_aout % 4 == 0)) && skinny_offsets_ok(g, false) &&
         (long long)g.M * g.ldz < (1LL << 31) && aligned16(g.z_out) && g.ldz % 4 == 0 &&
         (!g.soft_out || (aligned16(g.soft_out) && g.ld_soft % 4 == 0)) && (!g.noise.q || aligned16(g.noise.q));
}

static bool tall_ln_ok(const GemmArgs* probs, int count) {
  for (int i = 0; i < count; ++i) {
    const GemmArgs& g = probs[i];
    if (g.M < 1024 || g.epi != EPI_NONE || !g.a_out || g.K % 4 || g.K > 1024 || g.K < 4 || g.ksplitA < g.K ||
        g.lda % 4 || g.ld_aout % 4 || ((uintptr_t)g.A | (uintptr_t)g.a_out | (uintptr_t)g.ln_g | (uintptr_t)g.ln_b) & 15 ||
        (long long)g.M * std::max(g.lda, g.ld_aout) >= (1LL << 31))
      return false;
  }
  return true;
}
static void after_ln_rows(GemmArgs& g) {
  g.A = g.a_out; g.lda = g.ld_aout;
  g.ln_g = g.ln_b = nullptr; g.a_out = nullptr;
}

static void plan_build(GemmPlan& pl, GemmLayout lay, int amode, const GemmArgs* probs, int count) {
  if (count < 1 || count > 4) return plan_fail(pl, "gemm_launch: bad problem count %d", count);
  GemmArgs pp[4];
  if (lay == G_NT && amode == AM_LNSILU && tall_ln_ok(probs, count)) {
    for (int i = 0; i < count; ++i) {
      plan_step(pl, GF_LN_ROWS, 1 << i, (probs[i].M + 3) / 4, 1, 1, 256).kc = probs[i].K <= 256 ? 1 : 4;
      after_ln_rows(pp[i] = probs[i]);
    }
    pl.ln_pre = 1; probs = pp; amode = AM_PLAIN;
  }
  if (lay == G_NT && amode == AM_LNSILU && count == 1 && ln_sample_ok(probs[0])) {
    const GemmArgs& g = probs[0];
    GemmStep& st = plan_step(pl, GF_LN_SAMPLE, 1, dr_xcd_grid(dr_cdiv(g.M, LS_MT) * (g.N / LS_NT)), 1, 1, 256);
    st.bm = LS_MT; st.bn = LS_NT; st.kc = (g.K + 15) >> 4; st.amode = AM_LNSILU; st.vec = 1; st.epi = EPI_SAMPLE;
    st.lds = (int)ln_sample_lds_bytes(g.K);
    return;
  }
  PlanProbs q;
  for (int i = 0; i < count; ++i) {
    const GemmArgs& g = probs[i];
    if (g.epi == EPI_SAMPLE && (g.C < 1 || g.C > 32 || 32 % g.C != 0 || g.N != g.R * g.C))
      return plan_fail(pl, "gemm_launch: sampler epilogue needs C | 32 and N == R*C (C=%d R=%d N=%d)", g.C, g.R, g.N);
    if (g.epi == EPI_ACTOR && (g.N != 2 * g.na || g.na > 8))
      return plan_fail(pl, "gemm_launch: actor epilogue needs N == 2A <= 16");
    if (g.epi != EPI_NONE && (lay != G_NT || (amode != AM_PLAIN && amode != AM_LNSILU) || g.M > 4096 ||
                              !skinny_offsets_ok(g, false)))
      return plan_fail(pl, "gemm_launch: fused epilogues need the NT skinny path");
    q.add(&g, i);
  }
  for (int i = 0; i < count; ++i)
    if (probs[i].M < 0 || probs[i].N < 0 || probs[i].K < 0) return plan_fail(pl, "gemm_launch: negative dims");
  if (lay != G_NT) return plan_route(pl, AM_PLAIN, lay == G_TN, true, q);
  if (amode < AM_PLAIN || amode > AM_STEBWD) return plan_fail(pl, "gemm_launch: bad amode");
  const int maxM = tile_count(q, 16, 16).maxM;
  const bool r16 = maxM <= 4096 && skinny_tile_rows(q, amode, maxM, false) == 16;
  const int lim = r16 ? 1024 : 256;
  for (int i = 0; i < count && (amode == AM_LNBWD || amode == AM_STEBWD); ++i) {
    const GemmArgs& g = probs[i];
    const bool rows = g.K % 4 == 0 && g.K <= lim && g.lda % 4 == 0 && g.ld_pre % 4 == 0 && g.ldb % 4 == 0 &&
                      (((uintptr_t)g.A | (uintptr_t)g.pre | (uintptr_t)g.W) & 15) == 0;
    const int gl = g.C / 4;
    if (amode == AM_LNBWD && (!rows || (((uintptr_t)g.ln_g | (uintptr_t)g.ln_b) & 15)))
      return plan_fail(pl, "gemm_launch: AM_LNBWD needs K %% 4 == 0, K <= %d, 16-byte aligned rows (K=%d)", lim, g.K);
    if (amode == AM_STEBWD && (!rows || g.C < 4 || g.C % 4 || (gl & (gl - 1)) || gl > 64 || g.K % g.C || !r16))
      return plan_fail(pl, "gemm_launch: AM_STEBWD needs 16-row tiles (gemm_bwd_rows16), K %% C == 0, C/4 a power "
                           "of two, K <= %d, 16-byte aligned rows (K=%d C=%d)", lim, g.K, g.C);
  }
  plan_route(pl, amode, false, false, q);
}
GemmPlan gemm_plan(GemmLayout lay, int amode, const GemmArgs* probs, int count) {
  GemmPlan pl;
  pl.rc = DR_OK; pl.err[0] = 0; pl.ln_pre = 0; pl.nsteps = 0;
  plan_build(pl, lay, amode, probs, count);
  return pl;
}

int gemm_bwd_fusable(const GemmPlan& pl) {
  if (pl.rc != DR_OK || pl.nsteps > 1) return 0;
  return pl.nsteps == 0 ? 16 : pl.step[0].family == GF_SKINNY ? pl.step[0].bm : 0;
}

template <auto KERNEL>
static void lds_opt_in(int bytes) {
  static const bool raised = [bytes] {
    (void)hipFuncSetAttribute((const void*)KERNEL, hipFuncAttributeMaxDynamicSharedMemorySize, bytes);
    return true;
  }();
  (void)raised;
}
template <int MT, int NT, int AMODE, bool B_KN, int EPI>
static void launch_skinny(const GemmStep& st, const GemmBatch& gb, hipStream_t s) {
  constexpr auto kv = k_gemm_skinny<MT, NT, AMODE, B_KN, true, EPI>;
  constexpr auto ks = k_gemm_skinny<MT, NT, AMODE, B_KN, false, EPI>;
  if (st.lds > 64 * 1024) lds_opt_in<kv>(150 * 1024), lds_opt_in<ks>(150 * 1024);
  hipLaunchKernelGGL((st.vec ? kv : ks), dim3(st.gx, st.gy, st.gz), dim3(st.block), st.lds, s, gb, st.npack);
}
template <int AMODE, bool B_KN>
static void exec_skinny(const GemmStep& st, const GemmBatch& gb, hipStream_t s) {
#define DR_SK(mt, nt, e) launch_skinny<mt, nt, AMODE, B_KN, e>(st, gb, s)
  const bool r64 = st.bm == 64;
  if (st.epi == EPI_SAMPLE) return r64 ? DR_SK(64, 32, EPI_SAMPLE) : DR_SK(16, 32, EPI_SAMPLE);
  if (st.epi == EPI_ACTOR) return r64 ? DR_SK(64, 16, EPI_ACTOR) : DR_SK(16, 16, EPI_ACTOR);
  if (r64) return DR_SK(64, 16, EPI_NONE);
  if constexpr (AMODE == AM_LNBWD)
    if (st.bn == 48) return DR_SK(16, 48, EPI_NONE);
  return st.bn == 32 ? DR_SK(16, 32, EPI_NONE) : DR_SK(16, 16, EPI_NONE);
#undef DR_SK
}

template <int AMODE, bool A_KM, bool B_KN>
static void exec_mode(const GemmStep& st, const GemmBatch& gb, hipStream_t s) {
  if constexpr (!A_KM && AMODE != AM_CONV && AMODE != AM_CONV_SRC)
    if (st.family == GF_SKINNY) return exec_skinny<AMODE, B_KN>(st, gb, s);
  hipLaunchKernelGGL((st.bm == 64 ? k_gemm<64, 64, AMODE, A_KM, B_KN> : k_gemm<32, 32, AMODE, A_KM, B_KN>),
                     dim3(st.gx, st.gy, st.gz), dim3(st.block), 0, s, gb);
}
template <int BM, int BN, int KC, bool A_KM, bool B_KN, int NW = 4>
static void launch_tile2(const GemmStep& st, const GemmBatch& gb, hipStream_t s) {
  constexpr auto kv = k_gemm_tile<BM, BN, KC, A_KM, B_KN, true, NW>;
  constexpr auto ks = k_gemm_tile<BM, BN, KC, A_KM, B_KN, false, NW>;
  hipLaunchKernelGGL((st.vec ? kv : ks), dim3(st.gx, st.gy, st.gz), dim3(st.block), 0, s, gb, st.splits, st.npack);
}
template <int NK>
static void launch_ln_sample_nk(const GemmStep& st, const GemmArgs& g, hipStream_t s) {
  if (st.lds > 64 * 1024) lds_opt_in<k_ln_gemm_sample<NK>>((int)ln_sample_lds_bytes(16 * NK));
  hipLaunchKernelGGL(k_ln_gemm_sample<NK>, dim3(st.gx), dim3(st.block), st.lds, s, g);
}

static int exec_step(const GemmStep& st, const GemmBatch& gb, hipStream_t s) {
  const dim3 grid(st.gx, st.gy, st.gz), blk(st.block);
  const GemmArgs& g = gb.p[0];
  switch (st.family) {
    case GF_LN_ROWS:
      hipLaunchKernelGGL((st.kc == 1 ? k_ln_silu_rows<1> : k_ln_silu_rows<4>), grid, blk, 0, s, g.M, g.K, g.A,
                         (int)g.lda, g.ln_g, g.ln_b, g.a_out, (int)g.ld_aout);
      return dr_check_launch("ln_silu_rows");
    case GF_LN_SAMPLE: {
#define DR_LS(n) launch_ln_sample_nk<n>, launch_ln_sample_nk<n + 1>, launch_ln_sample_nk<n + 2>, launch_ln_sample_nk<n + 3>
      static void (*const nk[16])(const GemmStep&, const GemmArgs&, hipStream_t) = {DR_LS(1), DR_LS(5), DR_LS(9),
                                                                                    DR_LS(13)};
#undef DR_LS
      nk[st.kc - 1](st, g, s);
      return dr_check_launch("ln_gemm_sample");
    }
    case GF_S3_TALL:
      return op_gemm_nt_split3_ex(g.M, g.N, g.K, g.A, (int)g.lda, g.A2, (int)g.lda2, g.ksplitA < g.K ? g.ksplitA : g.K,
                                  g.wsplit, g.bias, g.act, g.Y, (int)g.ldy, g.accumulate, g.Y2, (int)g.ldy2,
                                  g.nsplitY < g.N ? g.nsplitY : INT_MAX, g.splitk_ws,
                                  g.splitk_ws ? (size_t)g.splitk_floats : 0, s, 0);
    case GF_TILE:
      if (st.bm == 32) launch_tile2<32, 32, 64, false, false, 4>(st, gb, s);
      else if (st.nw == 8) launch_tile2<64, 64, 64, false, false, 8>(st, gb, s);
      else if (st.a_km) launch_tile2<64, 64, 32, true, true>(st, gb, s);
      else if (st.b_kn) launch_tile2<64, 64, 32, false, true>(st, gb, s);
      else launch_tile2<64, 64, 32, false, false>(st, gb, s);
      break;
    case GF_TILE_B16:
      hipLaunchKernelGGL((st.bm == 32 ? k_gemm_tile_b16<32, 32, 4> : k_gemm_tile_b16<64, 64, 8>), grid, blk, 0, s, gb,
                         st.splits);
      break;
    case GF_SPLITK_FINISH: hipLaunchKernelGGL(k_splitk_finish, grid, blk, 0, s, gb, st.splits); break;
    case GF_WK: hipLaunchKernelGGL((k_gemm_wk<32, 32, 4, 2, 1>), grid, blk, 0, s, gb, 1, st.npack); break;
    case GF_WKS3:
      hipLaunchKernelGGL((st.a16    ? k_gemm_wks3<1, DR_WKS3_D, DR_WKS3_NW, DR_WKS3_FM_B16, true>
                          : st.bf16 ? k_gemm_wks3<1, DR_WKS3_D, DR_WKS3_NW, DR_WKS3_FM_B16>
                                    : k_gemm_wks3<3, DR_WKS3_D, DR_WKS3_NW, DR_WKS3_FM>),
                         grid, blk, 0, s, gb, st.npack);
      break;
    case GF_SKINNY:
    case GF_LEGACY:
      switch (st.amode) {
        case AM_LNSILU: exec_mode<AM_LNSILU, false, false>(st, gb, s); break;
        case AM_CONV: exec_mode<AM_CONV, false, false>(st, gb, s); break;
        case AM_CONV_SRC: exec_mode<AM_CONV_SRC, false, false>(st, gb, s); break;
        case AM_LNBWD: exec_mode<AM_LNBWD, false, false>(st, gb, s); break;
        case AM_STEBWD: exec_mode<AM_STEBWD, false, false>(st, gb, s); break;
        default:
          if (st.a_km) exec_mode<AM_PLAIN, true, true>(st, gb, s);
          else if (st.b_kn) exec_mode<AM_PLAIN, false, true>(st, gb, s);
          else exec_mode<AM_PLAIN, false, false>(st, gb, s);
      }
      break;
  }
  return DR_OK;
}

int gemm_launch(GemmLayout lay, int amode, const GemmArgs* probs, int count, hipStream_t s) {
  return gemm_run(gemm_plan(lay, amode, probs, count), probs, count, s);
}
int gemm_run(const GemmPlan& pl, const GemmArgs* probs, int count, hipStream_t s) {
  if (pl.rc != DR_OK) return dr_set_error("%s", pl.err), pl.rc;
  for (int k = 0; k < pl.nsteps; ++k) {
    const GemmStep& st = pl.step[k];
    GemmBatch gb;
    for (int i = 0, n = 0; i < count; ++i) {
      if (!(st.mask >> i & 1)) continue;
      GemmArgs& g = gb.p[n++] = probs[i];
      if (pl.ln_pre && st.family != GF_LN_ROWS) after_ln_rows(g);
      if (st.no_ws) g.splitk_ws = nullptr;
    }
    DR_TRY(exec_step(st, gb, s));
    if (st.family == GF_LN_SAMPLE) return DR_OK;
  }
  return dr_check_launch("gemm");
}

enum { GX_ALPHA, GX_ACT, GX_LDY2, GX_NSPLITY, GX_KSPLITB, GX_NSPLITB, GX_LD_ADD, GX_LD_PRE, GX_LD_SV, GX_LD_SOFT, GX_LD_MU,
       GX_LD_SIG, GX_LD_ACT, GX_GB_LDH, GX_GB_LDO, GX_GB_HD, GX_OHOW, GX_UNIMIX, GX_DET, GX_STEP, GX_LDB2, GX_COUNT = 24 };
enum { GP_Y2, GP_SV_GY, GP_SV_XH, GP_SOFT, GP_IDX, GP_ZVAL, GP_Q, GP_EPS, GP_MU, GP_SIG, GP_ACT, GP_GB_H, GP_GB_R, GP_GB_U,
       GP_GB_N, GP_GB_GHN, GP_GB_GI, GP_GB_GH, GP_GB_HO, GP_COUNT = 24 };
template <class PtrSource>
static GemmArgs hook_args(const int* v, PtrSource ptr, const double* num, void* const* xp) {
  const int fl = v[11];
  GemmArgs g = gemm_args();
  g.M = v[0]; g.N = v[1]; g.K = v[2]; g.C = v[8]; g.R = v[9]; g.na = v[10];
  g.bf16 = (fl >> 7) & 1; g.epi = (fl >> 8) & 3; g.out_conv = (fl >> 11) & 1; g.accumulate = (fl >> 13) & 1;
  g.A = ptr(0, 0, true); g.lda = v[3];
  g.A2 = ptr(1, 1, fl & 1); g.lda2 = v[4]; g.ksplitA = v[5];
  g.W = ptr(2, 2, true); g.ldb = v[6];
  g.Y = ptr(3, 3, true); g.ldy = v[7];
  g.ln_g = ptr(4, 4, fl & 2); g.ln_b = ptr(5, 5, fl & 2);
  g.a_out = ptr(6, 6, fl & 4); g.ld_aout = v[16];
  g.pre = ptr(7, 7, fl & 8); g.ld_pre = v[3];
  g.splitk_ws = ptr(8, -1, fl & 16); g.splitk_floats = v[12];
  g.wsplit = (const unsigned short*)ptr(9, 8, fl & 32); g.wsplit_np = v[13];
  g.A16 = (const unsigned short*)ptr(10, 9, fl & 64);
  g.W2 = ptr(11, -1, fl & 1024); g.ldb2 = v[6];
  g.addend = ptr(12, -1, fl & 4096); g.ld_add = v[7];
  g.bias = ptr(13, 10, fl & 16384);
  g.z_out = ptr(14, 11, g.epi == EPI_SAMPLE); g.ldz = v[7];
  if (num) {
    g.alpha = (float)num[GX_ALPHA]; g.act = (int)num[GX_ACT];
    g.ldy2 = (long long)num[GX_LDY2]; g.nsplitY = (int)num[GX_NSPLITY];
    g.ksplitB = (int)num[GX_KSPLITB]; g.nsplitB = (int)num[GX_NSPLITB]; g.ldb2 = (long long)num[GX_LDB2];
    g.ld_add = (long long)num[GX_LD_ADD]; g.ld_pre = (long long)num[GX_LD_PRE]; g.ld_sv = (long long)num[GX_LD_SV];
    g.ld_soft = (long long)num[GX_LD_SOFT]; g.ld_mu = (long long)num[GX_LD_MU]; g.ld_sig = (long long)num[GX_LD_SIG];
    g.ld_act = (long long)num[GX_LD_ACT];
    g.gb.ldh = (long long)num[GX_GB_LDH]; g.gb.ldo = (long long)num[GX_GB_LDO]; g.gb.Hd = (int)num[GX_GB_HD];
    g.oh = (int)num[GX_OHOW]; g.ow = 1;
    g.unimix = (float)num[GX_UNIMIX]; g.det = (int)num[GX_DET]; g.step = (int)num[GX_STEP];
  }
  if (xp) {
    auto f = [&](int k) { return (float*)xp[k]; };
    g.Y2 = f(GP_Y2); g.sv_gy = f(GP_SV_GY); g.sv_xh = f(GP_SV_XH);
    g.soft_out = f(GP_SOFT); g.idx_out = (int*)xp[GP_IDX]; g.zval_out = f(GP_ZVAL);
    g.noise.q = f(GP_Q); g.noise.eps = f(GP_EPS);
    g.mu_out = f(GP_MU); g.sig_out = f(GP_SIG); g.act_out = f(GP_ACT);
    g.gb.h = f(GP_GB_H); g.gb.r = f(GP_GB_R); g.gb.u = f(GP_GB_U); g.gb.n = f(GP_GB_N); g.gb.ghn = f(GP_GB_GHN);
    g.gb.gi = f(GP_GB_GI); g.gb.gh = f(GP_GB_GH); g.gb.ho = f(GP_GB_HO);
  }
  return g;
}
static int hook_steps(const GemmPlan& pl, int* out, int out_steps, char* msg, int msg_cap) {
  if (pl.rc != DR_OK) snprintf(msg, msg_cap, "%s", pl.err);
  static_assert(sizeof(GemmStep) == 21 * sizeof(int), "GemmStep is copied out as 21 ints");
  for (int k = 0; pl.rc == DR_OK && k < pl.nsteps && k < out_steps; ++k)
    memcpy(out + 21 * k, &pl.step[k], sizeof(GemmStep));
  return pl.rc != DR_OK ? -pl.rc : pl.nsteps;
}

extern "C" int dr_internal_gemm_plan(int lay, int amode, int count, const int* in, int* out, int out_steps, char* msg,
                                     int msg_cap) {
  GemmArgs pr[4];
  for (int i = 0; i < count && i < 4; ++i) {
    const int* v = in + 17 * i;
    auto ptr = [&](int slot, int nib, bool on) {
      const int mis = nib < 0 ? 0 : (v[14 + nib / 8] >> (4 * (nib % 8))) & 15;
      return on ? (float*)(((uintptr_t)(16 * i + slot + 1) << 32) + mis) : nullptr;
    };
    pr[i] = hook_args(v, ptr, nullptr, nullptr);
  }
  return hook_steps(gemm_plan((GemmLayout)lay, amode, pr, count), out, out_steps, msg, msg_cap);
}

extern "C" int dr_internal_gemm_run(int lay, int amode, int count, const int* in, void* const* ptrs, const double* num,
                                    void* const* xp, void* stream, int* out, int out_steps, char* msg, int msg_cap) {
  hipStream_t s = (hipStream_t)stream;
  GemmArgs pr[4];
  for (int i = 0; i < count && i < 4; ++i) {
    auto ptr = [&](int slot, int, bool on) { return on ? (float*)ptrs[15 * i + slot] : nullptr; };
    pr[i] = hook_args(in + 17 * i, ptr, num ? num + GX_COUNT * i : nullptr, xp ? xp + GP_COUNT * i : nullptr);
  }
  const GemmPlan pl = gemm_plan((GemmLayout)lay, amode, pr, count);
  const int n = hook_steps(pl, out, out_steps, msg, msg_cap);
  if (n < 0) return n;
  int rc = DR_OK;
  for (int i = 0; i < count && rc == DR_OK; ++i) {
    const GemmArgs& g = pr[i];
    if (g.wsplit && g.wsplit_np > 0 && g.N > 0 && g.K > 0) {
      if (g.wsplit_np == (g.N + 127) / 128 * 128) {
        rc = op_nt_repack_split3(g.N, g.K, g.W, (int)g.ldb, (void*)g.wsplit, s);
      } else {
        RepackJob j = rj_nt(g.N, g.K, g.W, (int)g.ldb, (void*)g.wsplit);
        j.c = g.wsplit_np; j.total = (long long)((g.K + 31) / 32) * 32 * g.wsplit_np;
        rc = op_repack_multi(&j, 1, s);
      }
    }
    if (rc == DR_OK && g.A16 && g.M > 0 && g.lda > 0) rc = op_to_bf16_2d(g.M, (int)g.lda, g.A, g.lda, (void*)g.A16, s);
  }
  if (rc == DR_OK) rc = gemm_run(pl, pr, count, s);
  if (rc != DR_OK) return snprintf(msg, msg_cap, "%s", dr_last_error()), -rc;
  return n;
}
```

dreamer_amd/csrc/gru.h:

```cpp
#pragma once
#include "common.h"

struct alignas(16) GruArgs {
  int B, Hd, R, C, A;
  const int* idx;
  const float* zval;
  const float* z;
  long long ldz;
  const float* a;
  long long lda;
  const float* h;
  long long ldh;
  const float* wt;
  const float* b_ih;
  const float* w_hh;
  const float* b_hh;
  float* hout;
  unsigned short* hout16;
  long long ldo;
  float *sr, *su, *sn, *sghn;
  float* gh_ws;
  int gh_ready;
};

int op_gru_fused(const GruArgs& g, hipStream_t s);
int op_zgather_add(int M, int N, int R, int C, const int* idx, const float* zval, const float* z, long long ldz,
                   const float* wt, long long ldw, const float* base, long long ldb, float* out, long long ldo,
                   hipStream_t s);
int op_transpose(int rows, int cols, const float* in, float* out, hipStream_t s);
struct TransposeJob {
  int rows, cols, ldo;
  const float* in;
  float* out;
};
#define DR_MAX_TJOBS 10
int op_transpose_multi(const TransposeJob* jobs, int n, hipStream_t s);
int op_onehot_index(int M, int R, int C, const float* z, long long ldz, int* idx, float* zval, hipStream_t s);
```

dreamer_amd/csrc/gru.hip:

```cpp
#include "gru.h"
#include "gemm.h"

#include <algorithm>

__global__ void k_transpose(int rows, int cols, const float* __restrict__ in, float* __restrict__ out) {
  __shared__ float tile[32][33];
  const int bx = blockIdx.x * 32, by = blockIdx.y * 32;
  const int tx = threadIdx.x & 31, ty = threadIdx.x >> 5;
  for (int k = ty; k < 32; k += 8) {
    const int r = by + k, c = bx + tx;
    tile[k][tx] = (r < rows && c < cols) ? in[(long long)r * cols + c] : 0.f;
  }
  __syncthreads();
  for (int k = ty; k < 32; k += 8) {
    const int c = bx + k, r = by + tx;
    if (c < cols && r < rows) out[(long long)c * rows + r] = tile[tx][k];
  }
}

int op_transpose(int rows, int cols, const float* in, float* out, hipStream_t s) {
  dim3 grid((cols + 31) / 32, (rows + 31) / 32);
  hipLaunchKernelGGL(k_transpose, grid, dim3(256), 0, s, rows, cols, in, out);
  return dr_check_launch("transpose");
}

struct TransposeBatch {
  TransposeJob j[DR_MAX_TJOBS];
};
__global__ void k_transpose_multi(TransposeBatch tb) {
  __shared__ float tile[32][33];
  const TransposeJob& J = tb.j[blockIdx.z];
  const int bx = blockIdx.x * 32, by = blockIdx.y * 32;
  if (bx >= J.cols || by >= J.rows) return;
  const int tx = threadIdx.x & 31, ty = threadIdx.x >> 5;
  for (int k = ty; k < 32; k += 8) {
    const int r = by + k, c = bx + tx;
    tile[k][tx] = (r < J.rows && c < J.cols) ? J.in[(long long)r * J.cols + c] : 0.f;
  }
  __syncthreads();
  for (int k = ty; k < 32; k += 8) {
    const int c = bx + k, r = by + tx;
    if (c < J.cols && r < J.rows) J.out[(long long)c * J.ldo + r] = tile[tx][k];
  }
}

int op_transpose_multi(const TransposeJob* jobs, int n, hipStream_t s) {
  if (n <= 0) return DR_OK;
  if (n > DR_MAX_TJOBS) {
    dr_set_error("transpose_multi: at most %d jobs", DR_MAX_TJOBS);
    return DR_E_INVALID;
  }
  TransposeBatch tb;
  int gx = 1, gy = 1;
  for (int i = 0; i < n; ++i) {
    tb.j[i] = jobs[i];
    gx = std::max(gx, (jobs[i].cols + 31) / 32);
    gy = std::max(gy, (jobs[i].rows + 31) / 32);
  }
  hipLaunchKernelGGL(k_transpose_multi, dim3(gx, gy, n), dim3(256), 0, s, tb);
  return dr_check_launch("transpose_multi");
}

__global__ void k_onehot_index(int M, int R, int C, const float* z, long long ldz, int* idx, float* zval) {
  const int i = blockIdx.x * blockDim.x + threadIdx.x;
  if (i >= M * R) return;
  const int m = i / R, g = i - m * R;
  const float* zz = z + (long long)m * ldz + g * C;
  int k = 0, nz = 0;
  float v = 0.f;
  for (int c = 0; c < C; ++c)
    if (zz[c] != 0.0f) {
      if (nz == 0) {
        k = c;
        v = zz[c];
      }
      ++nz;
    }
  idx[i] = nz > 1 ? -1 : k;
  zval[i] = nz > 1 ? 0.f : v;
}

int op_onehot_index(int M, int R, int C, const float* z, long long ldz, int* idx, float* zval, hipStream_t s) {
  if (M * R == 0) return DR_OK;
  hipLaunchKernelGGL(k_onehot_index, dim3((M * R + 255) / 256), dim3(256), 0, s, M, R, C, z, ldz, idx, zval);
  return dr_check_launch("onehot_index");
}

#ifndef GRU_MW
#define GRU_MW 4
#endif
#ifndef GRU_PRE
#define GRU_PRE 10
#endif
#define GRU_MAXR 32
#define GRU_MAXA 8

#ifdef DR_PHASE_TIMING
__device__ long long dr_tbuf_gru[1024 * DR_TS_SLOTS];
extern "C" int dr_debug_tbuf_gru(long long* out, int n) {
  const int rc = (int)hipMemcpyFromSymbol(out, HIP_SYMBOL(dr_tbuf_gru), (size_t)n * sizeof(long long));
  static long long zeros[1024 * DR_TS_SLOTS];
  return rc | (int)hipMemcpyToSymbol(HIP_SYMBOL(dr_tbuf_gru), zeros, sizeof(zeros));
}
#endif

__global__ __launch_bounds__(512) void k_gru_fused(GruArgs ga) {
  __shared__ GruArgs g;
  dr_stage_args(ga, g, threadIdx.x);
  const int Hd = dr_uni(g.Hd), B = dr_uni(g.B);
  const int R = dr_uni(g.R), C = dr_uni(g.C), A = dr_uni(g.A), L = R * C;
  const int tiles_j = (Hd + 15) / 16, tiles_m = (B + 15) / 16;
  const int lt = dr_xcd_tile(blockIdx.x, tiles_j * tiles_m);
  if (lt < 0) return;
  const int tj = lt / tiles_m, tm = lt - tj * tiles_m;
  const int m0 = tm * 16, j0 = tj * 16;
  const int tid = threadIdx.x, wave = tid >> 6, lane = tid & 63;
  DR_TS(dr_tbuf_gru, 0);

  __shared__ float red[GRU_MW][3][4][64];
  __shared__ float gi_s[16][3][16];
  __shared__ float gh_s[16][3][16];

  const float* h = dr_uni(g.h);
  if (wave < GRU_MW) {
    const float* whh = dr_uni(g.w_hh);
    const int ldh = dr_uni((int)g.ldh);
    const int r = lane & 15, q = lane >> 4;
    const int K = Hd;
    const int kw = ((K + GRU_MW * 16 - 1) / (GRU_MW * 16)) * 16;
    const int kb = wave * kw, ke = min(K, kb + kw);
    const int mrow = m0 + r, jrow = j0 + r;
    const bool mok = mrow < B, jok = jrow < Hd;
    f32x4 acc[3];
#pragma unroll
    for (int t = 0; t < 3; ++t) acc[t] = (f32x4){0.f, 0.f, 0.f, 0.f};
    if (h) {
      for (int kc = kb; kc < ke; kc += GRU_PRE * 16) {
        float4 ha[GRU_PRE], wb[GRU_PRE][3];
#pragma unroll
        for (int p = 0; p < GRU_PRE; ++p) {
          const int kq = kc + 16 * p + 4 * q;
          const bool live = kc + 16 * p < ke && kq < K;
          const bool oka = live && mok, okb = live && jok;
          ha[p] = dr_ld4(h, oka ? (unsigned)(mrow * ldh + kq) : 0u);
          if (!oka) ha[p] = make_float4(0.f, 0.f, 0.f, 0.f);
#pragma unroll
          for (int t = 0; t < 3; ++t) {
            wb[p][t] = dr_ld4(whh, okb ? (unsigned)((t * Hd + jrow) * K + kq) : 0u);
            if (!okb) wb[p][t] = make_float4(0.f, 0.f, 0.f, 0.f);
          }
        }
#pragma unroll
        for (int p = 0; p < GRU_PRE; ++p) {
          if (kc + 16 * p >= ke) break;
#pragma unroll
          for (int t = 0; t < 3; ++t) acc[t] = __builtin_amdgcn_mfma_f32_16x16x4f32(ha[p].x, wb[p][t].x, acc[t], 0, 0, 0);
#pragma unroll
          for (int t = 0; t < 3; ++t) acc[t] = __builtin_amdgcn_mfma_f32_16x16x4f32(ha[p].y, wb[p][t].y, acc[t], 0, 0, 0);
#pragma unroll
          for (int t = 0; t < 3; ++t) acc[t] = __builtin_amdgcn_mfma_f32_16x16x4f32(ha[p].z, wb[p][t].z, acc[t], 0, 0, 0);
#pragma unroll
          for (int t = 0; t < 3; ++t) acc[t] = __builtin_amdgcn_mfma_f32_16x16x4f32(ha[p].w, wb[p][t].w, acc[t], 0, 0, 0);
        }
      }
    }
#pragma unroll
    for (int t = 0; t < 3; ++t)
#pragma unroll
      for (int e = 0; e < 4; ++e) red[wave][t][e][lane] = acc[t][e];
    DR_TS(dr_tbuf_gru, 1);
  } else {
    const int x = tid - GRU_MW * 64;
    if (x < 192) {
      const int j4 = x & 3, t = (x >> 2) % 3, ml = x / 12;
      const int m = m0 + ml, jj = j0 + 4 * j4;
      const bool live = m < B && jj < Hd;
      const int* idx = dr_uni(g.idx);
      const float* zval = dr_uni(g.zval);
      const float* wt = dr_uni(g.wt);
      const float* act = dr_uni(g.a);
      const int lda = dr_uni((int)g.lda);
      const unsigned ldw = 3u * Hd;
      const unsigned col = (unsigned)(t * Hd + jj);
      int iv[GRU_MAXR];
      float zv[GRU_MAXR];
#pragma unroll
      for (int u4 = 0; u4 < GRU_MAXR / 4; ++u4) {
        const bool ok = live && 4 * u4 < R;
        const unsigned e = ok ? (unsigned)(m * R + 4 * u4) : 0u;
        const dr_f4 i4f = *(const DR_GLOBAL dr_f4*)((const DR_GLOBAL char*)idx + (e << 2));
// ... 357 lines not shown
```

dreamer_amd/csrc/ops.h:

```cpp
#pragma once
#include "common.h"

int op_gru_fwd(int B, int Hd, const float* gi, const float* gh, const float* h, long long ldh, float* hout,
               long long ldo, float* sr, float* su, float* sn, float* sghn, hipStream_t s);
int op_gru_bwd(int B, int Hd, const float* g_hp, long long ldg, const float* h, long long ldh, const float* sr,
               const float* su, const float* sn, const float* sghn, float* g_gi, float* g_gh, float* gh_out,
               long long ldo, int accumulate, hipStream_t s);
int op_sample(int M, int R, int C, const float* logits, long long ldl, const dr_noise* nz, int step, float* z,
              long long ldz, int* idx, float* soft, long long lds, hipStream_t s);
int op_softmax_ste_bwd(int M, int R, int C, const float* gz, long long ldg, const float* soft, long long lds,
                       float* g_logits, hipStream_t s);
int op_ln_silu_bwd(int M, int K, const float* gx, long long ldgx, const float* pre, long long ldp,
                   const float* gamma, const float* beta, float* g_pre, long long ldgp, float* gy, float* xhat,
                   hipStream_t s, unsigned short* g_pre16 = nullptr);
struct ColsumJob {
  int N;
  const float* X; long long ldx;
  const float* Y; long long ldy;
  float* out;
};
#define DR_MAX_CSJOBS 8
int op_colsum_multi(int M, const ColsumJob* jobs, int n, hipStream_t s);
int op_colsum(int M, int N, const float* X, long long ldx, const float* Y, long long ldy, float* out, int accumulate,
              hipStream_t s);
int op_bucket_value(int M, int nb, const float* logits, long long ldl, const float* buckets, float* out,
                    long long ostride, hipStream_t s);
int op_sigmoid(int M, const float* x, long long ldx, float* out, long long ostride, hipStream_t s);
int op_actor_head(int M, int A, const float* mu_raw, long long ldm, const float* ls_raw, long long ldl,
                  const dr_noise* nz, int step, int deterministic, float* a, long long lda, float* mu,
                  long long ldmu, float* sigma, long long lds, float* eps_save, hipStream_t s);
int op_actor_head_bwd_x(int M, int A, int N, const float* g_a, long long ldga, const float* g_mu_l,
                        const float* g_sig_l, long long ldgl, const float* a, long long lda, const float* ls_raw,
                        long long ldl, const float* eps, float* g_heads, long long ldh, const float* wt, float* gx,
                        long long ldx, hipStream_t s);
int op_actor_head_bwd(int M, int A, const float* g_a, long long ldga, const float* g_mu_l, const float* g_sig_l,
                      long long ldgl, const float* a, long long lda, const float* sigma, long long lds,
                      const float* ls_raw, long long ldl, const float* eps, float* g_heads, long long ldh,
                      hipStream_t s);
int op_conv_repack(int cout, int cin, const float* w, float* wr, hipStream_t s);
int op_fill(long long n, float* x, float v, hipStream_t s);
int op_copy2d(float* dst, long long dp, const float* src, long long sp, long long width, long long rows,
              hipStream_t s);
struct Copy2dJob {
  float* dst;
  long long dp;
  const float* src;
  long long sp, width, rows;
  int v4, pad_;
};
#define DR_COPY_MAX 4
int op_copy2d_multi(const Copy2dJob* jobs, int n, hipStream_t s);
int op_mean(int n, const float* x, float* out, hipStream_t s);

int op_vec_gather(int n, int nb, int D, const dr_frames* src, float* X, hipStream_t s);
```

dreamer_amd/csrc/ops.hip:

```cpp
#include <stdarg.h>

#include <algorithm>
#include <stdio.h>

#include "ops.h"

static thread_local char g_err[512] = "";

void dr_set_error(const char* fmt, ...) {
  va_list ap;
  va_start(ap, fmt);
  vsnprintf(g_err, sizeof(g_err), fmt, ap);
  va_end(ap);
}

int dr_check_launch(const char* what) {
  hipError_t e = hipGetLastError();
  if (e != hipSuccess) {
    dr_set_error("%s: %s", what, hipGetErrorString(e));
    return DR_E_HIP;
  }
  return DR_OK;
}

// ... 391 lines not shown
extern "C" int dr_bucket_value(int M, int nb, const float* logits, const float* buckets, float* out,
                               hipStream_t stream) {
  return op_bucket_value(M, nb, logits, nb, buckets, out, 1, stream);
}

__global__ void k_sigmoid(int M, const float* x, long long ldx, float* out, long long ostride) {
  const int i = blockIdx.x * blockDim.x + threadIdx.x;
  if (i >= M) return;
  out[(long long)i * ostride] = 1.0f / (1.0f + expf(-x[(long long)i * ldx]));
}

int op_sigmoid(int M, const float* x, long long ldx, float* out, long long ostride, hipStream_t s) {
  if (M == 0) return DR_OK;
  hipLaunchKernelGGL(k_sigmoid, dim3(dr_cdiv(M, 256)), dim3(256), 0, s, M, x, ldx, out, ostride);
  return dr_check_launch("sigmoid");
}

__global__ void k_actor_head(int M, int A, const float* __restrict__ mu_raw, long long ldm,
                             const float* __restrict__ ls_raw, long long ldl, dr_noise nz, int step, int det,
                             float* a, long long lda, float* mu, long long ldmu, float* sigma, long long lds,
                             float* eps_save) {
  const int i = blockIdx.x * blockDim.x + threadIdx.x;
  if (i >= M * A) return;
  const int m = i / A, k = i - m * A;
  const float muv = mu_raw[(long long)m * ldm + k];
  const float ls = fminf(fmaxf(ls_raw[(long long)m * ldl + k], -5.0f), 2.0f);
  const float sg = dr_softplus(ls) + 1e-3f;
  float av;
  if (det) {
    av = tanhf(muv);
  } else {
    float e;
    if (nz.eps) e = nz.eps[((long long)step * M + m) * A + k];
    else e = dr_normal(nz.rng, (uint32_t)(nz.stream + step), (uint32_t)(nz.row0 + m), (uint32_t)k);
    if (eps_save) eps_save[i] = e;
    av = tanhf(muv + e * sg);
  }
  if (a) a[(long long)m * lda + k] = av;
  if (mu) mu[(long long)m * ldmu + k] = muv;
  if (sigma) sigma[(long long)m * lds + k] = sg;
}

int op_actor_head(int M, int A, const float* mu_raw, long long ldm, const float* ls_raw, long long ldl,
                  const dr_noise* nz, int step, int deterministic, float* a, long long lda, float* mu,
                  long long ldmu, float* sigma, long long lds, float* eps_save, hipStream_t s) {
  if (M * A == 0) return DR_OK;
  hipLaunchKernelGGL(k_actor_head, dim3(dr_cdiv(M * A, 256)), dim3(256), 0, s, M, A, mu_raw, ldm, ls_raw, ldl, *nz,
                     step, deterministic, a, lda, mu, ldmu, sigma, lds, eps_save);
  return dr_check_launch("actor_head");
}

__global__ void k_actor_head_bwd(int M, int A, const float* g_a, long long ldga, const float* g_mu_l,
                                 const float* g_sig_l, long long ldgl, const float* a, long long lda,
                                 const float* sigma, long long lds, const float* ls_raw, long long ldl,
                                 const float* eps, float* g_heads, long long ldh) {
  const int i = blockIdx.x * blockDim.x + threadIdx.x;
  if (i >= M * A) return;
  const int m = i / A, k = i - m * A;
  float gmu = g_mu_l ? g_mu_l[(long long)m * ldgl + k] : 0.0f;
  float gsg = g_sig_l ? g_sig_l[(long long)m * ldgl + k] : 0.0f;
  if (g_a) {
    const float av = a[(long long)m * lda + k];
    const float gp = g_a[(long long)m * ldga + k] * (1.0f - av * av);
    gmu = gmu + gp;
    gsg = gsg + gp * eps[i];
  }
  const float lr = ls_raw[(long long)m * ldl + k];
  const float lc = fminf(fmaxf(lr, -5.0f), 2.0f);
  float gls = 0.0f;
  if (lr >= -5.0f && lr <= 2.0f) {
    const float ez = expf(lc);
    gls = (lc > 20.0f) ? gsg : gsg * ez / (ez + 1.0f);
  }
  g_heads[(long long)m * ldh + k] = gmu;
  g_heads[(long long)m * ldh + A + k] = gls;
}

int op_actor_head_bwd(int M, int A, const float* g_a, long long ldga, const float* g_mu_l, const float* g_sig_l,
                      long long ldgl, const float* a, long long lda, const float* sigma, long long lds,
                      const float* ls_raw, long long ldl, const float* eps, float* g_heads, long long ldh,
                      hipStream_t s) {
  if (M * A == 0) return DR_OK;
  hipLaunchKernelGGL(k_actor_head_bwd, dim3(dr_cdiv(M * A, 256)), dim3(256), 0, s, M, A, g_a, ldga, g_mu_l, g_sig_l,
                     ldgl, a, lda, sigma, lds, ls_raw, ldl, eps, g_heads, ldh);
  return dr_check_launch("actor_head_bwd");
}

__global__ __launch_bounds__(256) void k_actor_head_bwd_x(int M, int A, int N, const float* g_a, long long ldga,
                                                          const float* g_mu_l, const float* g_sig_l, long long ldgl,
                                                          const float* a, long long lda, const float* ls_raw,
                                                          long long ldl, const float* eps, float* g_heads,
                                                          long long ldh, const float* wt, float* gx, long long ldx) {
  __shared__ float gh[16][2 * 8];
  const int m0 = blockIdx.y * 16, n0 = blockIdx.x * 64, tid = threadIdx.x;
  const int nl = tid & 63, mq = tid >> 6;
  const int n = n0 + nl;
  float w[16];
#pragma unroll
  for (int k = 0; k < 16; ++k) w[k] = (k < 2 * A && n < N) ? wt[(long long)n * 2 * A + k] : 0.f;
  if (tid < 16 * A) {
    const int ml = tid / A, k = tid - ml * A, m = m0 + ml;
    float gmu = 0.f, gls = 0.f;
    if (m < M) {
      gmu = g_mu_l ? g_mu_l[(long long)m * ldgl + k] : 0.0f;
      float gsg = g_sig_l ? g_sig_l[(long long)m * ldgl + k] : 0.0f;
      if (g_a) {
        const float av = a[(long long)m * lda + k];
        const float gp = g_a[(long long)m * ldga + k] * (1.0f - av * av);
        gmu = gmu + gp;
        gsg = gsg + gp * eps[(long long)m * A + k];
      }
      const float lr = ls_raw[(long long)m * ldl + k];
      const float lc = fminf(fmaxf(lr, -5.0f), 2.0f);
      if (lr >= -5.0f && lr <= 2.0f) {
        const float ez = expf(lc);
        gls = (lc > 20.0f) ? gsg : gsg * ez / (ez + 1.0f);
      }
      if (blockIdx.x == 0) {
        g_heads[(long long)m * ldh + k] = gmu;
        g_heads[(long long)m * ldh + A + k] = gls;
      }
    }
    gh[ml][k] = gmu;
    gh[ml][A + k] = gls;
  }
  __syncthreads();
  if (n >= N) return;
#pragma unroll
  for (int i = 0; i < 4; ++i) {
    const int ml = 4 * mq + i, m = m0 + ml;
    if (m >= M) break;
    float v = 0.f;
#pragma unroll
    for (int k = 0; k < 16; ++k)
      if (k < 2 * A) v = fmaf(gh[ml][k], w[k], v);
    gx[(long long)m * ldx + n] = v;
  }
}

int op_actor_head_bwd_x(int M, int A, int N, const float* g_a, long long ldga, const float* g_mu_l,
                        const float* g_sig_l, long long ldgl, const float* a, long long lda, const float* ls_raw,
                        long long ldl, const float* eps, float* g_heads, long long ldh, const float* wt, float* gx,
                        long long ldx, hipStream_t s) {
  if (M == 0) return DR_OK;
  if (A > 8) {
    dr_set_error("actor_head_bwd_x: at most 8 actions");
    return DR_E_INVALID;
  }
  hipLaunchKernelGGL(k_actor_head_bwd_x, dim3(dr_cdiv(N, 64), dr_cdiv(M, 16)), dim3(256), 0, s, M, A, N, g_a, ldga,
                     g_mu_l, g_sig_l, ldgl, a, lda, ls_raw, ldl, eps, g_heads, ldh, wt, gx, ldx);
  return dr_check_launch("actor_head_bwd_x");
}

__global__ void k_lambda_returns(int B, int H, const float* r, const float* c, const float* V, float gamma,
                                 float lam, float lam_c, float* R) {
  const int b = blockIdx.x * blockDim.x + threadIdx.x;
  if (b >= B) return;
  const float* rb = r + (long long)b * H;
  const float* cb = c + (long long)b * H;
  const float* vb = V + (long long)b * (H + 1);
  float* Rb = R + (long long)b * H;
  float nxt = rb[H - 1] + (gamma * cb[H - 1]) * vb[H];
  Rb[H - 1] = nxt;
  for (int t = H - 2; t >= 0; --t) {
    const float v = rb[t] + (gamma * cb[t]) * ((lam_c * vb[t + 1]) + (lam * nxt));
    Rb[t] = v;
    nxt = v;
  }
}

extern "C" int dr_lambda_returns(int B, int H, const float* r, const float* c, const float* V, float gamma,
                                 float lam, float* R, hipStream_t stream) {
  if (B <= 0 || H <= 0) {
    dr_set_error("lambda_returns: bad dims B=%d H=%d", B, H);
    return DR_E_INVALID;
  }
  const float lam_c = (float)(1.0 - (double)lam);
  hipLaunchKernelGGL(k_lambda_returns, dim3(dr_cdiv(B, 64)), dim3(64), 0, stream, B, H, r, c, V, gamma, lam, lam_c,
                     R);
  return dr_check_launch("lambda_returns");
}

#define DR_SORT_MAX 16384

__device__ float torch_lerp(float a, float b, float w) {
  return (w < 0.5f) ? a + w * (b - a) : b - (b - a) * (1.0f - w);
}

__device__ __forceinline__ unsigned f2key(float x) {
  const unsigned u = __float_as_uint(x);
  return (u & 0x80000000u) ? ~u : (u | 0x80000000u);
}
__device__ __forceinline__ float key2f(unsigned k) {
  return __uint_as_float((k & 0x80000000u) ? (k & 0x7fffffffu) : ~k);
}

__global__ __launch_bounds__(1024) void k_update_S_select(int n, const float* R, float* S, float* norm_out) {
  __shared__ unsigned hist[4][256];
  __shared__ unsigned prefix[4], want[4];
  __shared__ int bad;
  const float r95 = 0.95f * (float)(n - 1), r05 = 0.05f * (float)(n - 1);
  if (threadIdx.x == 0) {
    bad = 0;
    want[0] = (unsigned)(int)r95;
    want[1] = (unsigned)(int)ceilf(r95);
    want[2] = (unsigned)(int)r05;
    want[3] = (unsigned)(int)ceilf(r05);
  }
  if (threadIdx.x < 4) prefix[threadIdx.x] = 0u;
  for (int pass = 0; pass < 4; ++pass) {
    const int shift = 24 - 8 * pass;
    const unsigned hi_mask = pass == 0 ? 0u : (0xffffffffu << (shift + 8));
    for (int i = threadIdx.x; i < 4 * 256; i += blockDim.x) (&hist[0][0])[i] = 0u;
    __syncthreads();
    unsigned pf[4];
#pragma unroll
    for (int t = 0; t < 4; ++t) pf[t] = prefix[t];
    for (int i = threadIdx.x; i < n; i += blockDim.x) {
      const float x = R[i];
      if (pass == 0 && !isfinite(x)) bad = 1;
      const unsigned k = f2key(x);
      const unsigned bin = (k >> shift) & 255u;
#pragma unroll
      for (int t = 0; t < 4; ++t)
        if ((k & hi_mask) == pf[t]) atomicAdd(&hist[t][bin], 1u);
    }
    __syncthreads();
    if (threadIdx.x < 4) {
      const int t = threadIdx.x;
      unsigned below = 0u, w = want[t];
      int b = 0;
      for (; b < 255; ++b) {
        const unsigned c = hist[t][b];
        if (below + c > w) break;
        below += c;
      }
      prefix[t] = pf[t] | ((unsigned)b << shift);
      want[t] = w - below;
    }
    __syncthreads();
  }
  if (threadIdx.x == 0) {
    float s = *S;
    if (!bad) {
      const float q95 = torch_lerp(key2f(prefix[0]), key2f(prefix[1]), r95 - (float)(int)r95);
      const float q05 = torch_lerp(key2f(prefix[2]), key2f(prefix[3]), r05 - (float)(int)r05);
      const float range = fmaxf(q95 - q05, 1.0f);
      s = 0.99f * s + 0.01f * range;
      *S = s;
    }
    if (norm_out) *norm_out = fmaxf(s, 1.0f);
  }
}

template <int VPT>
__global__ __launch_bounds__(1024) void k_update_S_reg(int n, const float* R, float* S, float* norm_out) {
  __shared__ unsigned hist[4][256];
  __shared__ unsigned prefix[4], want[4];
  __shared__ int bad;
  const float r95 = 0.95f * (float)(n - 1), r05 = 0.05f * (float)(n - 1);
  const int tid = threadIdx.x, wave = tid >> 6, lane = tid & 63;
  if (tid == 0) {
    bad = 0;
    want[0] = (unsigned)(int)r95;
    want[1] = (unsigned)(int)ceilf(r95);
    want[2] = (unsigned)(int)r05;
    want[3] = (unsigned)(int)ceilf(r05);
  }
  if (tid < 4) prefix[tid] = 0u;
  unsigned key[VPT];
  bool nonfinite = false;
#pragma unroll
  for (int v = 0; v < VPT; ++v) {
    const int i = tid + 1024 * v;
    const float x = R[i < n ? i : 0];
    nonfinite = nonfinite || (i < n && !isfinite(x));
    key[v] = f2key(x);
  }
  __syncthreads();
  if (nonfinite) bad = 1;
  for (int pass = 0; pass < 4; ++pass) {
    const int shift = 24 - 8 * pass;
    const unsigned hi_mask = pass == 0 ? 0u : (0xffffffffu << (shift + 8));
    (&hist[0][0])[tid] = 0u;
    __syncthreads();
    unsigned pf[4];
#pragma unroll
    for (int t = 0; t < 4; ++t) pf[t] = prefix[t];
#pragma unroll
    for (int v = 0; v < VPT; ++v) {
      if (tid + 1024 * v < n) {
        const unsigned k = key[v], bin = (k >> shift) & 255u;
#pragma unroll
        for (int t = 0; t < 4; ++t)
          if ((k & hi_mask) == pf[t]) atomicAdd(&hist[t][bin], 1u);
      }
    }
    __syncthreads();
    if (wave < 4) {
      const int t = wave;
      const unsigned w = want[t];
      const unsigned c0 = hist[t][4 * lane], c1 = hist[t][4 * lane + 1], c2 = hist[t][4 * lane + 2],
                     c3 = hist[t][4 * lane + 3];
      const unsigned sum = c0 + c1 + c2 + c3;
      unsigned inc = sum;
#pragma unroll
// ... 649 lines not shown
```

Measured before the change: 636,100 imagined latent-steps/s.

## Merge GRU input/hidden and actor-l0 backward GEMMs into segmented-K wks3 launches

In the imagination backward pass, the state-gradient GEMMs through the GRU input and hidden weights are merged with the actor first-layer backward GEMM. This uses concatenated transposed weights (K = 3*Hd + actor_h1) and a segmented-K A operand in the wks3 kernel. The action-gradient GEMM against the GRU input weights is folded into a new actor-head backward kernel that computes the dot products in-block. The goal is fewer kernel launches and fewer passes over the gradient outputs per timestep. The cost is extra weight transposes and split planes at prep, a new kernel template variant, and a per-element branch in the A load.

```diff
diff --git a/dreamer_amd/csrc/engine.hip b/dreamer_amd/csrc/engine.hip
--- a/dreamer_amd/csrc/engine.hip
+++ b/dreamer_amd/csrc/engine.hip
@@ -406,6 +406,8 @@
   unsigned short *ggi16, *ggh16, *gpre1a16;
   long long sk_n;
   float *tl6p, *tl3p, *tl0p, *twhh, *thead, *tl3a, *tl0a;
+  float *whs, *wzs;
+  void *s3whs, *s3wzs;
   void* tn;
   size_t tn_bytes;
   void* pd;
@@ -449,6 +451,10 @@
   w.thead = c.f((long long)2 * A * d->actor_h2);
   w.tl3a = c.f((long long)d->actor_h2 * d->actor_h1);
   w.tl0a = c.f((long long)d->actor_h1 * (Hd + L));
+  w.whs = c.f((long long)Hd * (3 * Hd + d->actor_h1));
+  w.wzs = c.f((long long)L * (3 * Hd + d->actor_h1));
+  w.s3whs = c.raw(op_nt_split3_ws_bytes(Hd, 3 * Hd + d->actor_h1));
+  w.s3wzs = c.raw(op_nt_split3_ws_bytes(L, 3 * Hd + d->actor_h1));
   w.gH = c.f(B1 * Hd);
   w.gZ = c.f(B1 * L);
   w.gA = c.f(BH * A);
@@ -800,6 +806,9 @@
                             const float* g_actions, const float* g_latents, const float* g_hiddens,
                             const void* tape, const dr_actor* gr, void* ws, size_t ws_bytes, hipStream_t s,
                             bool do_prep, bool do_main);
+static bool bwd_merged(const dr_dims* d, int B) {
+  return B >= 128 && (3 * d->hidden) % 8 == 0 && d->actor_h1 % 8 == 0 && d->precision != DR_PREC_BF16;
+}
 
 extern "C" int dr_imagine_bwd(const dr_dims* d, const dr_world_model* wm, const dr_actor* ac, int B, int H,
                               const float* latents, const float* hiddens, const float* actions,
@@ -862,7 +871,9 @@
   }
   {
     const int h1 = d->prior_h1, h2 = d->prior_h2;
-    TransposeJob tj[9] = {
+    const int Ks = 3 * Hd + a1;
+    const bool merged = bwd_merged(d, B);
+    TransposeJob tj[13] = {
         {L, h2, L, wm->prior.l6.w, w.tl6p},
         {h2, h1, h2, wm->prior.l3.w, w.tl3p},
         {h1, Hd, h1, wm->prior.l0.w, w.tl0p},
@@ -872,16 +883,24 @@
         {A, a2, 2 * A, ac->ls.w, w.thead + A},
         {a2, a1, a2, ac->l3.w, w.tl3a},
         {a1, Hd + L, a1, ac->l0.w, w.tl0a},
+        {3 * Hd, Hd, Ks, wm->w_hh, w.whs},
+        {a1, Hd, Ks, ac->l0.w, w.whs + 3 * Hd, Hd + L},
+        {3 * Hd, L, Ks, wm->w_ih, w.wzs, L + A},
+        {a1, L, Ks, ac->l0.w + Hd, w.wzs + 3 * Hd, Hd + L},
     };
-    DR_TRY(op_transpose_multi(tj, 9, s));
-    if (B >= 128 && (3 * Hd) % 8 == 0) {
+    DR_TRY(op_transpose_multi(tj, merged ? 13 : 9, s));
+    if (merged) {
+      DR_TRY(split_planes(L, Ks, w.wzs, Ks, w.s3wzs, s));
+      DR_TRY(split_planes(Hd, Ks, w.whs, Ks, w.s3whs, s));
+      DR_TRY(split_planes(Hd + L, a1, w.tl0a, a1, w.s3tl0a, s));
+    } else if (B >= 128 && (3 * Hd) % 8 == 0) {
       DR_TRY(split_planes(L + A, 3 * Hd, w.wt, 3 * Hd, w.s3wt, s));
       DR_TRY(split_planes(Hd, 3 * Hd, w.twhh, 3 * Hd, w.s3twhh, s));
-      if (d->actor_h1 % 8 == 0) DR_TRY(split_planes(Hd + L, d->actor_h1, w.tl0a, d->actor_h1, w.s3tl0a, s));
-    }
-  }
-  }
-  const bool planes = B >= 128 && (3 * Hd) % 8 == 0;
+      if (a1 % 8 == 0) DR_TRY(split_planes(Hd + L, a1, w.tl0a, a1, w.s3tl0a, s));
+    }
+  }
+  }
+  const bool planes = B >= 128 && (3 * Hd) % 8 == 0, merged = bwd_merged(d, B);
   if (!do_main) return DR_OK;
 
   bool looped = false;
@@ -928,7 +947,7 @@
       }
       DR_TRY(lnbwd_nt(B, Hd, h1, w.gx1, h1, tp.pre1p + (long long)t * B * h1, h1, wm->prior.n1, w.tl0p, gH_n, ldH, 1,
                       w.gp1, h1, nullptr, nullptr, nullptr, 0, INT_MAX, s, &ge));
-      if (t > 0) {
+      if (!merged && t > 0) {
         GemmArgs p[2];
         p[0] = bwd_nt(B, L + A, 3 * Hd, w.ggi, 3 * Hd, w.wt, gZ_t, ldL, 1);
         p[0].Y2 = w.gA + (long long)t * A; p[0].ldy2 = ldA; p[0].nsplitY = L;
@@ -942,27 +961,46 @@
           p[1].A16 = w.ggh16;
         }
         DR_TRY(gemm_launch(G_NT, AM_PLAIN, p, 2, s));
-      } else {
+      } else if (!merged) {
         DR_TRY(run(G_NT, AM_PLAIN, bwd_nt(B, A, 3 * Hd, w.ggi, 3 * Hd, w.wt + (long long)L * 3 * Hd, w.gA, ldA, 1), s));
       }
     }
     const long long ot = (long long)t * A;
     float* gh_t = w.gheads + (long long)t * 2 * A;
     const long long o2 = (long long)t * a2, o1 = (long long)t * a1;
-    DR_TRY(op_actor_head_bwd_x(B, A, a2, w.gA + ot, ldA, g_mus ? g_mus + ot : nullptr,
-                               g_sigmas ? g_sigmas + ot : nullptr, ldA, actions + ot, ldA, tp.ls_raw + ot, ldA,
-                               tp.eps + (long long)t * B * A, gh_t, (long long)H * 2 * A, w.thead, w.gx2a, a2, s));
+    if (merged && state_grad)
+      DR_TRY(op_actor_head_bwd_xga(B, A, a2, 3 * Hd, w.ggi, 3 * Hd, w.wt + (long long)L * 3 * Hd, 3 * Hd, w.gA + ot,
+                                   ldA, g_mus ? g_mus + ot : nullptr, g_sigmas ? g_sigmas + ot : nullptr, ldA,
+                                   actions + ot, ldA, tp.ls_raw + ot, ldA, tp.eps + (long long)t * B * A, gh_t,
+                                   (long long)H * 2 * A, w.thead, w.gx2a, a2, s));
+    else
+      DR_TRY(op_actor_head_bwd_x(B, A, a2, w.gA + ot, ldA, g_mus ? g_mus + ot : nullptr,
+                                 g_sigmas ? g_sigmas + ot : nullptr, ldA, actions + ot, ldA, tp.ls_raw + ot, ldA,
+                                 tp.eps + (long long)t * B * A, gh_t, (long long)H * 2 * A, w.thead, w.gx2a, a2, s));
     DR_TRY(lnbwd_nt(B, a1, a2, w.gx2a, a2, tp.pre2a + o2, lda2, ac->n4, w.tl3a, w.gx1a, a1, 0, w.gpre2a + o2, lda2,
                     w.gy2a + o2, w.xh2a + o2, nullptr, 0, INT_MAX, s));
     if (t > 0 && planes && a1 % 8 == 0) {
       const bool a16 = d->precision == DR_PREC_BF16 && lda1 % 8 == 0;
       DR_TRY(op_ln_silu_bwd(B, a1, w.gx1a, a1, tp.pre1a + o1, lda1, ac->n1.w, ac->n1.b, w.gpre1a + o1, lda1,
                             w.gy1a + o1, w.xh1a + o1, s, a16 ? w.gpre1a16 + o1 : nullptr));
-      GemmArgs g = bwd_nt(B, Hd + L, a1, w.gpre1a + o1, lda1, w.tl0a, gH_t, ldH, 1);
-      if (a16) g.A16 = w.gpre1a16 + o1;
-      g.Y2 = gZ_t; g.ldy2 = ldL; g.nsplitY = Hd;
-      wplanes(g, w.s3tl0a);
-      DR_TRY(run(G_NT, AM_PLAIN, g, s));
+      if (merged && state_grad) {
+        const int Ks = 3 * Hd + a1;
+        GemmArgs p[2];
+        p[0] = bwd_nt(B, L, Ks, w.ggi, 3 * Hd, w.wzs, gZ_t, ldL, 1);
+        p[1] = bwd_nt(B, Hd, Ks, w.ggh, 3 * Hd, w.whs, gH_t, ldH, 1);
+        wplanes(p[0], w.s3wzs);
+        wplanes(p[1], w.s3whs);
+        for (int i = 0; i < 2; ++i) {
+          p[i].A2 = w.gpre1a + o1; p[i].lda2 = lda1; p[i].ksplitA = 3 * Hd;
+        }
+        DR_TRY(gemm_launch(G_NT, AM_PLAIN, p, 2, s));
+      } else {
+        GemmArgs g = bwd_nt(B, Hd + L, a1, w.gpre1a + o1, lda1, w.tl0a, gH_t, ldH, 1);
+        if (a16) g.A16 = w.gpre1a16 + o1;
+        g.Y2 = gZ_t; g.ldy2 = ldL; g.nsplitY = Hd;
+        wplanes(g, w.s3tl0a);
+        DR_TRY(run(G_NT, AM_PLAIN, g, s));
+      }
     } else if (t > 0) {
       DR_TRY(lnbwd_nt(B, Hd + L, a1, w.gx1a, a1, tp.pre1a + o1, lda1, ac->n1, w.tl0a, gH_t, ldH, 1, w.gpre1a + o1,
                       lda1, w.gy1a + o1, w.xh1a + o1, gZ_t, ldL, Hd, s));
diff --git a/dreamer_amd/csrc/gemm.h b/dreamer_amd/csrc/gemm.h
--- a/dreamer_amd/csrc/gemm.h
+++ b/dreamer_amd/csrc/gemm.h
@@ -43,6 +43,7 @@
   GruBwdEpi gb;
   const unsigned short* wsplit; int wsplit_np, pad2_;
   const unsigned short* A16;
+  const unsigned short* A2_16;
 };
 
 enum { EPI_NONE = 0, EPI_SAMPLE = 1, EPI_ACTOR = 2 };
diff --git a/dreamer_amd/csrc/gemm.hip b/dreamer_amd/csrc/gemm.hip
--- a/dreamer_amd/csrc/gemm.hip
+++ b/dreamer_amd/csrc/gemm.hip
@@ -1713,7 +1713,7 @@
   return __builtin_bit_cast(unsigned, v);
 }
 
-template <int NTP, int D, int NW = 4, int FM = 2, bool A16 = false>
+template <int NTP, int D, int NW = 4, int FM = 2, bool A16 = false, bool SEG = false>
 __global__ __launch_bounds__(64 * NW) void k_gemm_wks3(GemmBatch gb, int npack) {
   static_assert(!A16 || NTP == 1, "bf16 A copies feed the one-term form only");
   constexpr int FN = 2, BM = 16 * FM, NTH = 64 * NW, NT4 = FM * FN * 256;
@@ -1734,6 +1734,9 @@
   const float* A = dr_uni(g.A);
   const unsigned short* A16p = dr_uni(g.A16);
   const int lda = dr_uni((int)g.lda);
+  const float* A2 = dr_uni(g.A2);
+  const unsigned short* A216p = dr_uni(g.A2_16);
+  const int lda2 = dr_uni((int)g.lda2), ksA = dr_uni(g.ksplitA);
   const unsigned short* wr = dr_uni(g.wsplit);
   const int Np = dr_uni(g.wsplit_np);
   constexpr int NEPI = (NT4 + NTH - 1) / NTH;
@@ -1754,6 +1757,11 @@
   unsigned oa[FM];
 #pragma unroll
   for (int i = 0; i < FM; ++i) oa[i] = (unsigned)(min(m0 + 16 * i + r, M - 1) * lda);
+  unsigned oa2[SEG ? FM : 1];
+  if constexpr (SEG) {
+#pragma unroll
+    for (int i = 0; i < FM; ++i) oa2[i] = (unsigned)(min(m0 + 16 * i + r, M - 1) * lda2);
+  }
   unsigned ob[FN];
 #pragma unroll
   for (int j = 0; j < FN; ++j) ob[j] = (unsigned)(n0 + 16 * j + r) * 32u + 8u * q;
@@ -1765,7 +1773,18 @@
     const unsigned kk = k < K ? (unsigned)k : 0u;
 #pragma unroll
     for (int i = 0; i < FM; ++i) {
-      if constexpr (A16) {
+      if constexpr (SEG) {
+        const bool s2 = (int)kk >= ksA;
+        const unsigned o = s2 ? oa2[i] + (kk - (unsigned)ksA) : oa[i] + kk;
+        if constexpr (A16) {
+          const DR_GLOBAL char* b = (const DR_GLOBAL char*)(s2 ? A216p : A16p);
+          ra16[sl][i] = *(const DR_GLOBAL wk_u32x4*)(b + (o << 1));
+        } else {
+          const DR_GLOBAL char* b = (const DR_GLOBAL char*)(s2 ? A2 : A);
+          ra[sl][i][0] = *(const DR_GLOBAL f32x4*)(b + (o << 2));
+          ra[sl][i][1] = *(const DR_GLOBAL f32x4*)(b + ((o + 4) << 2));
+        }
+      } else if constexpr (A16) {
         ra16[sl][i] = *(const DR_GLOBAL wk_u32x4*)((const DR_GLOBAL char*)A16p + ((oa[i] + kk) << 1));
       } else {
         ra[sl][i][0] = *(const DR_GLOBAL f32x4*)((const DR_GLOBAL char*)A + ((oa[i] + kk) << 2));
@@ -2296,13 +2315,15 @@
 }
 static bool b16_ok(const PlanProbs& q) { return chain_ok(q, true); }
 
+static bool wks3_seg(const GemmArgs& g) { return g.ksplitA < g.K; }
 static bool wks3_ok(const PlanProbs& q) {
   for (int i = 0; i < q.n; ++i) {
     const GemmArgs& g = q[i];
     if (!g.wsplit || g.wsplit_np < ((g.N + 31) & ~31) || g.K < 8 || !rows_aligned(g, 8, true, false) ||
-        ((uintptr_t)g.wsplit & 15) || g.ksplitA < g.K || g.W2 || g.epi != EPI_NONE || g.out_conv || g.M < 1 || g.N < 1 ||
+        ((uintptr_t)g.wsplit & 15) || g.W2 || g.epi != EPI_NONE || g.out_conv || g.M < 1 || g.N < 1 ||
         (long long)g.M * g.lda >= (1LL << 30) || (long long)((g.K + 31) / 32) * 3 * g.wsplit_np * 32 >= (1LL << 30))
       return false;
+    if (wks3_seg(g) && (!g.A2 || g.ksplitA < 8 || g.lda2 < 0 || (long long)g.M * g.lda2 >= (1LL << 30))) return false;
   }
   return true;
 }
@@ -2316,7 +2337,10 @@
   if (tc.maxt == 0) return;
   const int npack = q.n > 1 ? q.n : 0;
   bool a16 = family == GF_WKS3 && bf16;
-  for (int i = 0; i < q.n && a16; ++i) a16 = q[i].A16 && ((uintptr_t)q[i].A16 & 15) == 0 && q[i].lda % 8 == 0;
+  for (int i = 0; i < q.n && a16; ++i) {
+    a16 = q[i].A16 && ((uintptr_t)q[i].A16 & 15) == 0 && q[i].lda % 8 == 0;
+    if (a16 && wks3_seg(q[i])) a16 = q[i].A2_16 && ((uintptr_t)q[i].A2_16 & 15) == 0 && q[i].lda2 % 8 == 0;
+  }
   GemmStep& st = plan_step(pl, family, q.mask, dr_xcd_grid(npack ? tc.tot : tc.maxt), 1, 1, 64 * nw);
   st.bm = 16 * fm; st.bn = 32; st.nw = nw; st.vec = 1; st.bf16 = family == GF_WKS3 && bf16; st.a16 = a16;
   st.splits = 1; st.npack = npack; st.no_ws = no_ws;
@@ -2567,12 +2591,22 @@
       break;
     case GF_SPLITK_FINISH: hipLaunchKernelGGL(k_splitk_finish, grid, blk, 0, s, gb, st.splits); break;
     case GF_WK: hipLaunchKernelGGL((k_gemm_wk<32, 32, 4, 2, 1>), grid, blk, 0, s, gb, 1, st.npack); break;
-    case GF_WKS3:
-      hipLaunchKernelGGL((st.a16    ? k_gemm_wks3<1, DR_WKS3_D, DR_WKS3_NW, DR_WKS3_FM_B16, true>
-                          : st.bf16 ? k_gemm_wks3<1, DR_WKS3_D, DR_WKS3_NW, DR_WKS3_FM_B16>
-                                    : k_gemm_wks3<3, DR_WKS3_D, DR_WKS3_NW, DR_WKS3_FM>),
-                         grid, blk, 0, s, gb, st.npack);
+    case GF_WKS3: {
+      bool seg = false;
+      for (int i = 0, n = 0; i < 4; ++i)
+        if (st.mask >> i & 1) seg = wks3_seg(gb.p[n++]) || seg;
+      if (seg)
+        hipLaunchKernelGGL((st.a16    ? k_gemm_wks3<1, DR_WKS3_D, DR_WKS3_NW, DR_WKS3_FM_B16, true, true>
+                            : st.bf16 ? k_gemm_wks3<1, DR_WKS3_D, DR_WKS3_NW, DR_WKS3_FM_B16, false, true>
+                                      : k_gemm_wks3<3, DR_WKS3_D, DR_WKS3_NW, DR_WKS3_FM, false, true>),
+                           grid, blk, 0, s, gb, st.npack);
+      else
+        hipLaunchKernelGGL((st.a16    ? k_gemm_wks3<1, DR_WKS3_D, DR_WKS3_NW, DR_WKS3_FM_B16, true>
+                            : st.bf16 ? k_gemm_wks3<1, DR_WKS3_D, DR_WKS3_NW, DR_WKS3_FM_B16>
+                                      : k_gemm_wks3<3, DR_WKS3_D, DR_WKS3_NW, DR_WKS3_FM>),
+                           grid, blk, 0, s, gb, st.npack);
       break;
+    }
     case GF_SKINNY:
     case GF_LEGACY:
       switch (st.amode) {
@@ -2614,7 +2648,7 @@
 enum { GX_ALPHA, GX_ACT, GX_LDY2, GX_NSPLITY, GX_KSPLITB, GX_NSPLITB, GX_LD_ADD, GX_LD_PRE, GX_LD_SV, GX_LD_SOFT, GX_LD_MU,
        GX_LD_SIG, GX_LD_ACT, GX_GB_LDH, GX_GB_LDO, GX_GB_HD, GX_OHOW, GX_UNIMIX, GX_DET, GX_STEP, GX_LDB2, GX_COUNT = 24 };
 enum { GP_Y2, GP_SV_GY, GP_SV_XH, GP_SOFT, GP_IDX, GP_ZVAL, GP_Q, GP_EPS, GP_MU, GP_SIG, GP_ACT, GP_GB_H, GP_GB_R, GP_GB_U,
-       GP_GB_N, GP_GB_GHN, GP_GB_GI, GP_GB_GH, GP_GB_HO, GP_COUNT = 24 };
+       GP_GB_N, GP_GB_GHN, GP_GB_GI, GP_GB_GH, GP_GB_HO, GP_A2_16, GP_COUNT = 24 };
 template <class PtrSource>
 static GemmArgs hook_args(const int* v, PtrSource ptr, const double* num, void* const* xp) {
   const int fl = v[11];
@@ -2654,6 +2688,7 @@
     g.mu_out = f(GP_MU); g.sig_out = f(GP_SIG); g.act_out = f(GP_ACT);
     g.gb.h = f(GP_GB_H); g.gb.r = f(GP_GB_R); g.gb.u = f(GP_GB_U); g.gb.n = f(GP_GB_N); g.gb.ghn = f(GP_GB_GHN);
     g.gb.gi = f(GP_GB_GI); g.gb.gh = f(GP_GB_GH); g.gb.ho = f(GP_GB_HO);
+    if (g.A16 && g.A2) g.A2_16 = (const unsigned short*)xp[GP_A2_16];
   }
   return g;
 }
@@ -2703,6 +2738,8 @@
       }
     }
     if (rc == DR_OK && g.A16 && g.M > 0 && g.lda > 0) rc = op_to_bf16_2d(g.M, (int)g.lda, g.A, g.lda, (void*)g.A16, s);
+    if (rc == DR_OK && g.A2_16 && g.M > 0 && g.lda2 > 0)
+      rc = op_to_bf16_2d(g.M, (int)g.lda2, g.A2, g.lda2, (void*)g.A2_16, s);
   }
   if (rc == DR_OK) rc = gemm_run(pl, pr, count, s);
   if (rc != DR_OK) return snprintf(msg, msg_cap, "%s", dr_last_error()), -rc;
diff --git a/dreamer_amd/csrc/gru.h b/dreamer_amd/csrc/gru.h
--- a/dreamer_amd/csrc/gru.h
+++ b/dreamer_amd/csrc/gru.h
@@ -32,7 +32,8 @@
   int rows, cols, ldo;
   const float* in;
   float* out;
+  int ldi;
 };
-#define DR_MAX_TJOBS 10
+#define DR_MAX_TJOBS 16
 int op_transpose_multi(const TransposeJob* jobs, int n, hipStream_t s);
 int op_onehot_index(int M, int R, int C, const float* z, long long ldz, int* idx, float* zval, hipStream_t s);
diff --git a/dreamer_amd/csrc/gru.hip b/dreamer_amd/csrc/gru.hip
--- a/dreamer_amd/csrc/gru.hip
+++ b/dreamer_amd/csrc/gru.hip
@@ -35,7 +35,7 @@
   const int tx = threadIdx.x & 31, ty = threadIdx.x >> 5;
   for (int k = ty; k < 32; k += 8) {
     const int r = by + k, c = bx + tx;
-    tile[k][tx] = (r < J.rows && c < J.cols) ? J.in[(long long)r * J.cols + c] : 0.f;
+    tile[k][tx] = (r < J.rows && c < J.cols) ? J.in[(long long)r * (J.ldi ? J.ldi : J.cols) + c] : 0.f;
   }
   __syncthreads();
   for (int k = ty; k < 32; k += 8) {
diff --git a/dreamer_amd/csrc/ops.h b/dreamer_amd/csrc/ops.h
--- a/dreamer_amd/csrc/ops.h
+++ b/dreamer_amd/csrc/ops.h
@@ -33,6 +33,11 @@
                         const float* g_sig_l, long long ldgl, const float* a, long long lda, const float* ls_raw,
                         long long ldl, const float* eps, float* g_heads, long long ldh, const float* wt, float* gx,
                         long long ldx, hipStream_t s);
+int op_actor_head_bwd_xga(int M, int A, int N, int K, const float* ggi, long long ldg, const float* wact,
+                          long long ldw, float* g_a, long long ldga, const float* g_mu_l, const float* g_sig_l,
+                          long long ldgl, const float* a, long long lda, const float* ls_raw, long long ldl,
+                          const float* eps, float* g_heads, long long ldh, const float* wt, float* gx, long long ldx,
+                          hipStream_t s);
 int op_actor_head_bwd(int M, int A, const float* g_a, long long ldga, const float* g_mu_l, const float* g_sig_l,
                       long long ldgl, const float* a, long long lda, const float* sigma, long long lds,
                       const float* ls_raw, long long ldl, const float* eps, float* g_heads, long long ldh,
diff --git a/dreamer_amd/csrc/ops.hip b/dreamer_amd/csrc/ops.hip
--- a/dreamer_amd/csrc/ops.hip
+++ b/dreamer_amd/csrc/ops.hip
@@ -567,6 +567,124 @@
   return dr_check_launch("actor_head_bwd_x");
 }
 
+template <int AMAX>
+__global__ __launch_bounds__(256) void k_actor_head_bwd_xga(int M, int A, int N, int K, const float* ggi, long long ldg,
+                                                            const float* wact, long long ldw, float* g_a,
+                                                            long long ldga, const float* g_mu_l, const float* g_sig_l,
+                                                            long long ldgl, const float* a, long long lda,
+                                                            const float* ls_raw, long long ldl, const float* eps,
+                                                            float* g_heads, long long ldh, const float* wt, float* gx,
+                                                            long long ldx) {
+  __shared__ float dots[4][8];
+  __shared__ float gh[4][2 * 8];
+  const int m0 = blockIdx.x * 4, tid = threadIdx.x;
+  const int nl = tid & 63, ml = tid >> 6;
+  float wv[4][2 * AMAX];
+#pragma unroll
+  for (int c = 0; c < 4; ++c)
+#pragma unroll
+    for (int k = 0; k < 2 * AMAX; ++k)
+      wv[c][k] = wt[(long long)min(nl + 64 * c, N - 1) * 2 * A + min(k, 2 * A - 1)];
+  {
+    const int j = nl, m = min(m0 + ml, M - 1);
+    const float4* x4 = reinterpret_cast<const float4*>(ggi + (long long)m * ldg);
+    const float4* w4[AMAX];
+    float acc[AMAX];
+#pragma unroll
+    for (int k = 0; k < AMAX; ++k) {
+      w4[k] = reinterpret_cast<const float4*>(wact + (long long)min(k, A - 1) * ldw);
+      acc[k] = 0.f;
+    }
+    constexpr int U = 32 / AMAX;
+    const int K4 = K >> 2;
+    for (int k0 = j; k0 < K4; k0 += 64 * U) {
+      float4 x[U], w[AMAX][U];
+#pragma unroll
+      for (int u = 0; u < U; ++u) {
+        const bool ok = k0 + 64 * u < K4;
+        const int kc = ok ? k0 + 64 * u : j;
+        x[u] = x4[kc];
+        if (!ok) x[u] = make_float4(0.f, 0.f, 0.f, 0.f);
+#pragma unroll
+        for (int k = 0; k < AMAX; ++k) w[k][u] = w4[k][kc];
+      }
+#pragma unroll
+      for (int u = 0; u < U; ++u)
+#pragma unroll
+        for (int k = 0; k < AMAX; ++k) {
+          const float4 xv = x[u], wk = w[k][u];
+          acc[k] = fmaf(xv.w, wk.w, fmaf(xv.z, wk.z, fmaf(xv.y, wk.y, fmaf(xv.x, wk.x, acc[k]))));
+        }
+    }
+#pragma unroll
+    for (int k = 0; k < AMAX; ++k) {
+      const float v = group_sum(acc[k], 64);
+      if (j == 0 && k < A) dots[ml][k] = v;
+    }
+  }
+  __syncthreads();
+  if (tid < 4 * A) {
+    const int rl = tid / A, k = tid - rl * A, m = m0 + rl;
+    float gmu = 0.f, gls = 0.f;
+    if (m < M) {
+      gmu = g_mu_l ? g_mu_l[(long long)m * ldgl + k] : 0.0f;
+      float gsg = g_sig_l ? g_sig_l[(long long)m * ldgl + k] : 0.0f;
+      const float ga = g_a[(long long)m * ldga + k] + dots[rl][k];
+      g_a[(long long)m * ldga + k] = ga;
+      const float av = a[(long long)m * lda + k];
+      const float gp = ga * (1.0f - av * av);
+      gmu = gmu + gp;
+      gsg = gsg + gp * eps[(long long)m * A + k];
+      const float lr = ls_raw[(long long)m * ldl + k];
+      const float lc = fminf(fmaxf(lr, -5.0f), 2.0f);
+      if (lr >= -5.0f && lr <= 2.0f) {
+        const float ez = expf(lc);
+        gls = (lc > 20.0f) ? gsg : gsg * ez / (ez + 1.0f);
+      }
+      g_heads[(long long)m * ldh + k] = gmu;
+      g_heads[(long long)m * ldh + A + k] = gls;
+    }
+    gh[rl][k] = gmu;
+    gh[rl][A + k] = gls;
+  }
+  __syncthreads();
+  const int m = m0 + ml;
+  if (m >= M) return;
+#pragma unroll
+  for (int c = 0; c < 4; ++c) {
+    const int n = nl + 64 * c;
+    float v = 0.f;
+#pragma unroll
+    for (int k = 0; k < 2 * AMAX; ++k)
+      if (k < 2 * A) v = fmaf(gh[ml][k], wv[c][k], v);
+    if (n < N) gx[(long long)m * ldx + n] = v;
+  }
+  for (int n = nl + 256; n < N; n += 64) {
+    float v = 0.f;
+#pragma unroll
+    for (int k = 0; k < 16; ++k)
+      if (k < 2 * A) v = fmaf(gh[ml][k], wt[(long long)n * 2 * A + k], v);
+    gx[(long long)m * ldx + n] = v;
+  }
+}
+
+int op_actor_head_bwd_xga(int M, int A, int N, int K, const float* ggi, long long ldg, const float* wact,
+                          long long ldw, float* g_a, long long ldga, const float* g_mu_l, const float* g_sig_l,
+                          long long ldgl, const float* a, long long lda, const float* ls_raw, long long ldl,
+                          const float* eps, float* g_heads, long long ldh, const float* wt, float* gx, long long ldx,
+                          hipStream_t s) {
+  if (M == 0) return DR_OK;
+  if (A < 1 || A > 8 || K % 4 != 0 || ldg % 4 != 0 || ldw % 4 != 0 || ((uintptr_t)ggi & 15) ||
+      ((uintptr_t)wact & 15) || !g_a) {
+    dr_set_error("actor_head_bwd_xga: at most 8 actions, 16-byte rows of K % 4 == 0 floats");
+    return DR_E_INVALID;
+  }
+  hipLaunchKernelGGL((A <= 4 ? k_actor_head_bwd_xga<4> : k_actor_head_bwd_xga<8>), dim3(dr_cdiv(M, 4)), dim3(256), 0, s,
+                     M, A, N, K, ggi, ldg, wact, ldw, g_a, ldga, g_mu_l, g_sig_l, ldgl, a, lda, ls_raw, ldl, eps, g_heads,
+                     ldh, wt, gx, ldx);
+  return dr_check_launch("actor_head_bwd_xga");
+}
+
 __global__ void k_lambda_returns(int B, int H, const float* r, const float* c, const float* V, float gamma,
                                  float lam, float lam_c, float* R) {
   const int b = blockIdx.x * blockDim.x + threadIdx.x;
```

Measured after the change: 640,000 imagined latent-steps/s (median of 6 runs). No clear change (+0.6%).
